# lawfuyang/ToyRenderer

Hardware: AMD Instinct MI355X
Metric: Gmeshlets/s culled (whole node), 100M meshlets (higher is better)
Workload: dtype f32

## Files before the change

toyrenderer_amd/csrc/host/nvrhi_lite.h:

```cpp
#pragma once

#include "HostProfile.h"

#include <atomic>
#include <cstdint>
#include <cstdio>
#include <cstdlib>
#include <memory>
#include <stdexcept>
#include <string>
#include <utility>
#include <vector>

#include "../../../include/trhip.h"

#define check(expr)                                                                          \
    do {                                                                                     \
        if (!(expr)) {                                                                       \
            std::fprintf(stderr, "check failed: %s (%s:%d)\n", #expr, __FILE__, __LINE__);   \
            std::abort();                                                                    \
        }                                                                                    \
    } while (0)

namespace nvrhi
// ... 316 lines not shown
    }
    void setPushConstants(const void* data, size_t bytes) { m_Push.assign((const uint8_t*)data, (const uint8_t*)data + bytes); }
    void dispatch(uint32_t gx, uint32_t gy = 1, uint32_t gz = 1)
    {
        std::vector<trhip_binding> b = flatten();
        HOST_PROFILE_SCOPE("trhip_cmd_dispatch (record)");
        throwIfFailed(trhip_cmd_dispatch(m_Native, m_State.pipeline.c_str(), b.data(), (uint32_t)b.size(),
                                         m_Push.empty() ? nullptr : m_Push.data(), (uint32_t)m_Push.size(), gx, gy, gz), "ICommandList::dispatch");
        m_Push.clear();
    }
    void dispatchIndirect(uint32_t offsetBytes)
    {
        check(m_State.indirectParams);
        std::vector<trhip_binding> b = flatten();
        HOST_PROFILE_SCOPE("trhip_cmd_dispatch_indirect (record)");
        throwIfFailed(trhip_cmd_dispatch_indirect(m_Native, m_State.pipeline.c_str(), b.data(), (uint32_t)b.size(),
                                                  m_Push.empty() ? nullptr : m_Push.data(), (uint32_t)m_Push.size(),
                                                  m_State.indirectParams->native(), offsetBytes), "ICommandList::dispatchIndirect");
        m_Push.clear();
    }
    void beginTimerQuery(ITimerQuery* q) { keep(q); throwIfFailed(trhip_cmd_begin_timer(m_Native, q->native()), "ICommandList::beginTimerQuery"); }
    void endTimerQuery(ITimerQuery* q) { q->m_Recorded = true; throwIfFailed(trhip_cmd_end_timer(m_Native, q->native()), "ICommandList::endTimerQuery"); }
    void beginPipelineStatisticsQuery(IPipelineStatisticsQuery* q) { keep(q); throwIfFailed(trhip_cmd_begin_pipeline_stats(m_Native, q->native()), "ICommandList::beginPipelineStatisticsQuery"); }
    void endPipelineStatisticsQuery(IPipelineStatisticsQuery* q) { q->m_Recorded = true; throwIfFailed(trhip_cmd_end_pipeline_stats(m_Native, q->native()), "ICommandList::endPipelineStatisticsQuery"); }
    void beginMarker(const char* name) { throwIfFailed(trhip_cmd_begin_marker(m_Native, name), "ICommandList::beginMarker"); }
    void endMarker() { throwIfFailed(trhip_cmd_end_marker(m_Native), "ICommandList::endMarker"); }

private:
    void keep(IResource* r) { if (r) m_Keep.emplace_back(r); }
    std::vector<trhip_binding> flatten() const
    {
        std::vector<trhip_binding> out;
        out.reserve(m_State.bindings.bindings.size());
        for (const BindingSetItem& i : m_State.bindings.bindings) {
            trhip_binding b{};
            b.type = i.type; b.slot = i.slot; b.baseMip = i.baseMip;
            if (i.buffer) b.resource = i.buffer->native();
            else if (i.texture) b.resource = i.texture->native();
            else if (i.table) b.resource = i.table->native();
            out.push_back(b);
        }
        return out;
    }

    trhip_cmdlist m_Native;
    ComputeState m_State;
    std::vector<uint8_t> m_Push;
    std::vector<ResourceHandle> m_Keep;
};
using CommandListHandle = RefCountPtr<ICommandList>;

namespace utils
{
struct ScopedMarker
{
    ScopedMarker(ICommandList* cl, const char* name) : m_Cl(cl) { m_Cl->beginMarker(name); }
    ~ScopedMarker() { m_Cl->endMarker(); }
    ICommandList* m_Cl;
};
}

class IDevice : public IResource
{
public:
    explicit IDevice(trhip_device d) : m_Native(d) {}
    ~IDevice() override { destroyQueues(); trhip_device_destroy(m_Native); }
    trhip_device native() const { return m_Native; }
    trhip_device queueDevice(CommandQueue queue)
    {
        if (queue != CommandQueue::Compute) return m_Native;
        if (!m_ComputeNative) {
            throwIfFailed(trhip_stream_create(m_DeviceIndex, &m_ComputeStream), "IDevice: compute-queue stream");
            throwIfFailed(trhip_device_create_on_stream(m_DeviceIndex, m_ComputeStream, &m_ComputeNative), "IDevice: compute-queue device");
        }
        return m_ComputeNative;
    }

    HeapHandle createHeap(const HeapDesc& d)
    {
        trhip_heap h = nullptr;
        throwIfFailed(trhip_heap_create(m_Native, d.capacity, &h), "IDevice::createHeap");
        return HeapHandle(new IHeap(h, d));
    }
    BufferHandle createBuffer(const BufferDesc& d)
    {
        trhip_buffer_desc n{};
        n.byteSize = d.byteSize; n.structStride = d.structStride; n.canHaveUAVs = d.canHaveUAVs; n.isDrawIndirectArgs = d.isDrawIndirectArgs;
        n.isVirtual = d.isVirtual; n.isVolatileConstant = d.isVolatile && d.isConstantBuffer; n.debugName = d.debugName.c_str();
        trhip_buffer b = nullptr;
        throwIfFailed(trhip_buffer_create(m_Native, &n, &b), "IDevice::createBuffer");
        return BufferHandle(new IBuffer(b, d));
    }
    TextureHandle createTexture(const TextureDesc& d)
    {
        trhip_texture_desc n{};
        n.width = d.width; n.height = d.height; n.mipLevels = d.mipLevels; n.isUAV = (d.isUAV ? 1u : 0u) | (d.isRenderTarget ? TRHIP_TEXTURE_RENDER_TARGET : 0u); n.isVirtual = d.isVirtual; n.debugName = d.debugName.c_str();
        n.format = d.format == Format::R16_FLOAT ? TRHIP_FORMAT_R16_FLOAT : d.format == Format::RG32_UINT ? TRHIP_FORMAT_RG32_UINT
                 : d.format == Format::RG16_FLOAT ? TRHIP_FORMAT_RG16_FLOAT : d.format == Format::RGBA32_UINT ? TRHIP_FORMAT_RGBA32_UINT
                 : d.format == Format::R11G11B10_FLOAT ? TRHIP_FORMAT_R11G11B10_FLOAT : d.format == Format::R8_UNORM ? TRHIP_FORMAT_R8_UNORM
                 : d.format == Format::R8_UINT ? TRHIP_FORMAT_R8_UINT : d.format == Format::RGBA8_UNORM ? TRHIP_FORMAT_RGBA8_UNORM
                 : d.format == Format::SRGBA8_UNORM ? TRHIP_FORMAT_SRGBA8_UNORM : d.format == Format::R10G10B10A2_UNORM ? TRHIP_FORMAT_R10G10B10A2_UNORM
                 : d.format == Format::RGBA16_FLOAT ? TRHIP_FORMAT_RGBA16_FLOAT : TRHIP_FORMAT_R32_FLOAT;
        trhip_texture t = nullptr;
        if (d.dimension == kTexture2DArray) throwIfFailed(trhip_texture_create_array(m_Native, &n, d.arraySize, &t), "IDevice::createTexture (array)");
        else throwIfFailed(trhip_texture_create(m_Native, &n, &t), "IDevice::createTexture");
        return TextureHandle(new ITexture(t, d));
    }
    SamplerHandle createSampler(const SamplerDesc& d) { return SamplerHandle(new ISampler(d)); }
    DescriptorTableHandle createDescriptorTable(uint32_t capacity)
    {
        trhip_texture_table t = nullptr;
        throwIfFailed(trhip_texture_table_create(m_Native, capacity, &t), "IDevice::createDescriptorTable");
        return DescriptorTableHandle(new IDescriptorTable(t));
    }
    void writeDescriptorTable(IDescriptorTable* table, uint32_t index, ITexture* t) { throwIfFailed(trhip_texture_table_set(table->native(), index, t->native()), "IDevice::writeDescriptorTable"); }
    MemoryRequirements getBufferMemoryRequirements(IBuffer* b)
    {
        MemoryRequirements r;
        throwIfFailed(trhip_buffer_memory_requirements(b->native(), &r.size, &r.alignment), "IDevice::getBufferMemoryRequirements");
        return r;
    }
    MemoryRequirements getTextureMemoryRequirements(ITexture* t)
    {
        MemoryRequirements r;
        throwIfFailed(trhip_texture_memory_requirements(t->native(), &r.size, &r.alignment), "IDevice::getTextureMemoryRequirements");
        return r;
    }
    bool bindBufferMemory(IBuffer* b, IHeap* h, uint64_t off) { throwIfFailed(trhip_buffer_bind_memory(b->native(), h->native(), off), "IDevice::bindBufferMemory"); return true; }
    bool bindTextureMemory(ITexture* t, IHeap* h, uint64_t off) { throwIfFailed(trhip_texture_bind_memory(t->native(), h->native(), off), "IDevice::bindTextureMemory"); return true; }
    CommandListHandle createCommandList(CommandQueue queue = CommandQueue::Graphics)
    {
        trhip_cmdlist cl = nullptr;
        throwIfFailed(trhip_cmd_create(queueDevice(queue), &cl), "IDevice::createCommandList");
        return CommandListHandle(new ICommandList(cl, queue));
    }
    uint64_t executeCommandLists(ICommandList* const* lists, size_t n, CommandQueue queue = CommandQueue::Graphics)
    {
        std::vector<trhip_cmdlist> v;
        for (size_t i = 0; i < n; ++i) { check(lists[i]->m_Queue == queue); v.push_back(lists[i]->native()); }
        throwIfFailed(trhip_queue_execute(queueDevice(queue), v.data(), (uint32_t)v.size()), "IDevice::executeCommandLists");
        return ++m_LastInstance[(size_t)queue];
    }
    uint64_t executeCommandList(ICommandList* cl) { return executeCommandLists(&cl, 1, cl->m_Queue); }
    void queueWaitForCommandList(CommandQueue waitQueue, CommandQueue executionQueue, uint64_t instance)
    {
        if (waitQueue == executionQueue) return;
        check(instance == m_LastInstance[(size_t)executionQueue]);
        trhip_device producer = queueDevice(executionQueue);
        void*& ev = m_QueueEvents[(size_t)executionQueue][instance % kQueueEvents];
        if (!ev) throwIfFailed(trhip_event_create(m_DeviceIndex, &ev), "IDevice::queueWaitForCommandList: event");
        throwIfFailed(trhip_device_join_side_stream(producer), "IDevice::queueWaitForCommandList: join");
        throwIfFailed(trhip_event_record(ev, trhip_device_stream(producer)), "IDevice::queueWaitForCommandList: record");
        throwIfFailed(trhip_stream_wait_event(trhip_device_stream(queueDevice(waitQueue)), ev), "IDevice::queueWaitForCommandList: wait");
    }
    uint64_t lastInstance(CommandQueue queue) const { return m_LastInstance[(size_t)queue]; }
    bool hasComputeQueue() const { return m_ComputeNative != nullptr; }
    void setDeviceIndex(int index) { m_DeviceIndex = index; }
    void waitForIdle()
    {
        throwIfFailed(trhip_device_wait_idle(m_Native), "IDevice::waitForIdle");
        if (m_ComputeNative) throwIfFailed(trhip_device_wait_idle(m_ComputeNative), "IDevice::waitForIdle (compute queue)");
    }
    void destroyQueues()
    {
        for (auto& q : m_QueueEvents) for (void*& e : q) { if (e) trhip_event_destroy(e); e = nullptr; }
        if (m_ComputeNative) { trhip_device_destroy(m_ComputeNative); m_ComputeNative = nullptr; }
        if (m_ComputeStream) { trhip_stream_destroy(m_ComputeStream); m_ComputeStream = nullptr; }
    }
    void runGarbageCollection() {}
    TimerQueryHandle createTimerQuery()
    {
        trhip_timer t = nullptr;
        throwIfFailed(trhip_timer_create(m_Native, &t), "IDevice::createTimerQuery");
        return TimerQueryHandle(new ITimerQuery(t));
    }
    float getTimerQueryTime(ITimerQuery* q)
    {
        if (!q || !q->m_Recorded) return 0.0f;
        float ms = 0.0f;
        if (trhip_timer_get_ms(q->native(), &ms) != TRHIP_OK) return 0.0f;
        return ms * 1e-3f;
    }
    void resetTimerQuery(ITimerQuery* q) { if (q) q->m_Recorded = false; }
    PipelineStatisticsQueryHandle createPipelineStatisticsQuery()
    {
        trhip_pipeline_stats q = nullptr;
        throwIfFailed(trhip_pipeline_stats_create(m_Native, &q), "IDevice::createPipelineStatisticsQuery");
        return PipelineStatisticsQueryHandle(new IPipelineStatisticsQuery(q));
    }
    PipelineStatistics getPipelineStatistics(IPipelineStatisticsQuery* q)
    {
        PipelineStatistics s;
        if (!q || !q->m_Recorded) return s;
        if (trhip_pipeline_stats_get(q->native(), reinterpret_cast<trhip_pipeline_statistics*>(&s)) != TRHIP_OK) return PipelineStatistics{};
        return s;
    }

private:
    static constexpr size_t kQueueEvents = 16;
    trhip_device m_Native;
    trhip_device m_ComputeNative = nullptr;
    void* m_ComputeStream = nullptr;
    int m_DeviceIndex = 0;
    uint64_t m_LastInstance[(size_t)CommandQueue::Count] = {};
    void* m_QueueEvents[(size_t)CommandQueue::Count][kQueueEvents] = {};
};
using DeviceHandle = RefCountPtr<IDevice>;

}
```

toyrenderer_amd/csrc/instance_cache.hip.h:

```cpp
#pragma once

#include <hip/hip_runtime.h>

#include "ShaderInterop.h"

struct InstanceCullCache
{
    const float4* sphere;
    const float4* world;
    const float* maxScale;
    const uint32_t* numLODs;
    const uint2* lodInfo;
    const float* error;
    const float4* localSphere;
    uint64_t stride;

    __host__ __device__ const uint2& lod(uint32_t id, uint32_t l) const { return lodInfo[(uint64_t)l * stride + id]; }
    __host__ __device__ const float& err(uint32_t id, uint32_t l) const { return error[(uint64_t)l * stride + id]; }
};

constexpr uint64_t kInstanceCacheBytesPerInstance = 64 + 16 + 4 + 4 + 3 * 4 * interop::kMaxNumMeshLODs + 16;

inline InstanceCullCache instanceCacheLayout(void* base, uint64_t n)
{
    char* p = (char*)base;
    InstanceCullCache c;
    c.world = (const float4*)p;             p += 64 * n;
    c.sphere = (const float4*)p;            p += 16 * n;
    c.maxScale = (const float*)p;           p += 4 * n;
    c.numLODs = (const uint32_t*)p;         p += 4 * n;
    c.lodInfo = (const uint2*)p;            p += 8ull * interop::kMaxNumMeshLODs * n;
    c.error = (const float*)p;              p += 4ull * interop::kMaxNumMeshLODs * n;
    c.localSphere = (const float4*)p;
    c.stride = n;
    return c;
}

__device__ __forceinline__ void instanceCacheWriteTransformPart(const InstanceCullCache& c, uint32_t i, float4 w0, float4 w1, float4 w2, float4 w3, float4 sph,
                                                                float4* worldOut = nullptr)
{
    const cm::M43 W = { { w0.x, w0.y, w0.z }, { w1.x, w1.y, w1.z }, { w2.x, w2.y, w2.z }, { w3.x, w3.y, w3.z } };
    const float ms = cm::maxScale(W.r0, W.r1, W.r2);
    const cm::F3 wc = cm::mulPoint({ sph.x, sph.y, sph.z }, W);
    const_cast<float4*>(c.sphere)[i] = make_float4(wc.x, wc.y, wc.z, sph.w * ms);
    float4* wr = worldOut ? worldOut : const_cast<float4*>(c.world) + 4ull * i;
    wr[0] = make_float4(w0.x, w0.y, w0.z, w1.x);
    wr[1] = make_float4(w1.y, w1.z, w2.x, w2.y);
    wr[2] = make_float4(w2.z, w3.x, w3.y, w3.z);
    wr[3] = make_float4(ms, 0.f, 0.f, 0.f);
    const_cast<float*>(c.maxScale)[i] = ms;
}
```

toyrenderer_amd/csrc/k_basepass_as.hip:

```cpp
#include <algorithm>
#include <cstdlib>
#include <string>
#include <type_traits>

#if defined(TR_STAMPS) || defined(TR_COUNT_SLOW) || defined(TR_COUNT_PATHS)
__device__ unsigned long long g_stampSums[8];
#define g_pathCount (g_stampSums + 4)
#endif
#include <atomic>
#include <memory>
#include <mutex>
#include <unordered_map>

#include "cull_math.hip.h"
#include "instance_cache.hip.h"
#include "meshlet_exact.hip.h"
#include "trhip_internal.h"

using namespace interop;

namespace
{

constexpr uint32_t kBlock = 256;
// ... 1101 lines not shown

void emitListBuild(const trhip::DispatchCtx& ctx, const MeshletCullArgs& a, const char* prefix, bool side, const void* argsBase)
{
    auto emit = [&](const std::string& name, std::function<int(hipStream_t)> fn) {
        if (side) ctx.emitSide(name.c_str(), std::move(fn), { { a.listGroups ? (const void*)a.listGroups : argsBase, false }, { a.visMask, false }, { a.visibleList, true }, { a.drawArgs, true } });
        else ctx.emit(name.c_str(), std::move(fn));
    };
    if (!side && a.recordCapacity <= kCompactMaxTiles * kCompactTile) {
        const uint32_t tiles = (a.recordCapacity + kCompactTile - 1) / kCompactTile;
        const size_t words = (size_t)kCompactMaxTiles * kStatusStride * 2 + 4;
        uint32_t* mem = (uint32_t*)ctx.scratch(words * 4);
        if (mem && ctx.cl->recordClearWords(mem, words, 0, true) == TRHIP_OK) {
            unsigned long long* status = (unsigned long long*)mem;
            uint32_t* ticket = mem + kCompactMaxTiles * kStatusStride * 2;
            uint32_t grid = ctx.computeUnits();
            if (grid > tiles) grid = tiles;
            if (grid == 0) grid = 1;
            emit(std::string(prefix) + "compact", [a, status, ticket, grid](hipStream_t s) {
                TRHIP_LAUNCH(visCompactKernel, dim3(grid), dim3(kCompactThreads), 0, s, a, status, ticket);
                return trhip::launchStatus("visCompactKernel"); });
            return;
        }
    }
    const uint32_t needBlocks = (a.maxBatches + kWaves - 1) / kWaves;
    uint32_t gridSmall = ctx.computeUnits() * 8u;
    if (gridSmall > needBlocks) gridSmall = needBlocks;
    if (gridSmall == 0) gridSmall = 1;
    const std::string p = prefix;
    const uint32_t supers = (a.maxBatches >> kSuperShift) + 1u;
    emit(p + "count", [a, supers](hipStream_t s) {
        TRHIP_LAUNCH(visCountKernel, dim3(supers), dim3(kCountThreads), 0, s, a);
        return trhip::launchStatus("visCountKernel"); });
    emit(p + "scan", [a](hipStream_t s) {
        TRHIP_LAUNCH(visSuperScanKernel, dim3(1), dim3(1024), 0, s, a);
        return trhip::launchStatus("visSuperScanKernel"); });
    emit(p + "expand", [a, gridSmall](hipStream_t s) {
        TRHIP_LAUNCH(visExpandKernel, dim3(gridSmall), dim3(kBlock), 0, s, a);
        return trhip::launchStatus("visExpandKernel"); });
}

template <bool F, bool O, bool C>
void launchCull(const MeshletCullArgs& a, uint32_t grid, bool table, hipStream_t s)
{
    if (O && table) TRHIP_LAUNCH((meshletCullKernel<F, O, C, true>), dim3(grid), dim3(kCullBlock), 0, s, a);
    else TRHIP_LAUNCH((meshletCullKernel<F, O, C, false>), dim3(grid), dim3(kCullBlock), 0, s, a);
}

constexpr uint64_t kStreamBytesPerMeshlet = 20;
__host__ __device__ inline MeshletCullStream meshletStreamLayout(void* mem, uint64_t numMeshlets)
{
    const uint64_t coneAt = (numMeshlets * 16u + 255u) & ~255ull;
    return { reinterpret_cast<const float4*>(mem), reinterpret_cast<const uint32_t*>(reinterpret_cast<char*>(mem) + coneAt) };
}
inline uint64_t meshletStreamBytes(uint64_t numMeshlets) { return ((numMeshlets * 16u + 255u) & ~255ull) + numMeshlets * 4u; }

__global__ __launch_bounds__(256) void meshletStreamKernel(const MeshletData* __restrict__ meshlets, uint64_t n, MeshletCullStream out)
{
    const uint64_t stride = (uint64_t)gridDim.x * 256u;
    for (uint64_t i = (uint64_t)blockIdx.x * 256u + threadIdx.x; i < n; i += stride) {
        const float4* p = reinterpret_cast<const float4*>(meshlets + i);
        const float4 sphere = p[0];
        const uint32_t cone = __float_as_uint(p[1].x);
        const_cast<float4*>(out.sphere)[i] = sphere;
        const_cast<uint32_t*>(out.cone)[i] = cone;
    }
}

int meshletStreamLaunchBuild(trhip_buffer_t* meshlets, hipStream_t s)
{
    const trhip::Stamp from = { meshlets->version };
    if (meshlets->cullStream.current(from)) return TRHIP_OK;
    const uint64_t n = meshlets->byteSize / sizeof(MeshletData);
    const uint64_t blocks = (n + 255u) / 256u;
    TRHIP_LAUNCH(meshletStreamKernel, dim3((uint32_t)(blocks < 65536u ? (blocks ? blocks : 1u) : 65536u)), dim3(256), 0, s,
                       (const MeshletData*)meshlets->ptr, n, meshletStreamLayout(meshlets->cullStream.ptr, n));
    meshlets->cullStream.markBuilt(from);
    return trhip::launchStatus("meshletStreamKernel");
}

int recordASMain(trhip::DispatchCtx& ctx)
{
    const BasePassConstants* k = (const BasePassConstants*)ctx.constants(0, sizeof(BasePassConstants));
    TRHIP_REQUIRE(k, "%s: constant buffer b0 (BasePassConstants, 256 bytes) missing", ctx.shaderName);
    trhip_buffer_t* instances = ctx.buffer(TRHIP_BIND_STRUCTURED_SRV, 0);
    trhip_buffer_t* meshData = ctx.buffer(TRHIP_BIND_STRUCTURED_SRV, 2);
    trhip_buffer_t* meshlets = ctx.buffer(TRHIP_BIND_STRUCTURED_SRV, 4);
    trhip_buffer_t* records = ctx.buffer(TRHIP_BIND_STRUCTURED_SRV, 7);
    trhip_texture_t* hzb = ctx.texture(TRHIP_BIND_TEXTURE_SRV, 8);
    trhip_buffer_t* visMask = ctx.buffer(TRHIP_BIND_STRUCTURED_UAV, 0);
    trhip_buffer_t* visList = ctx.buffer(TRHIP_BIND_STRUCTURED_UAV, 1);
    trhip_buffer_t* drawArgs = ctx.buffer(TRHIP_BIND_STRUCTURED_UAV, 2);
    TRHIP_REQUIRE(instances && meshData && meshlets && records, "%s: needs SRVs t0, t2, t4, t7 (BasePassRenderers.cpp:463-479)", ctx.shaderName);
    TRHIP_REQUIRE(visMask && visList && drawArgs, "%s: needs UAVs u0 (visMask), u1 (visibleList), u2 (drawArgs)", ctx.shaderName);
    TRHIP_REQUIRE(ctx.indirect, "%s: launched by dispatchMeshIndirect (BasePassRenderers.cpp:497-502): use dispatch_indirect", ctx.shaderName);
    TRHIP_REQUIRE(instances->byteSize % sizeof(BasePassInstanceConstants) == 0, "%s: instance buffer size is not a multiple of 144", ctx.shaderName);
    TRHIP_REQUIRE(meshlets->byteSize % sizeof(MeshletData) == 0, "%s: meshlet buffer size is not a multiple of 32", ctx.shaderName);
    TRHIP_REQUIRE(drawArgs->byteSize >= 12, "%s: drawArgs buffer smaller than 12 bytes", ctx.shaderName);

    MeshletCullArgs a;
    memset(&a, 0, sizeof a);
    a.k = *k;
    const bool occlusion = (k->m_CullingFlags & kCullingFlagOcclusionCullingEnable) != 0;
    const bool useTable = occlusion && ctx.variant == 0 && records->byteSize / sizeof(MeshletAmplificationData) >= trhip::tableMinGroups();
    int rc = TRHIP_OK;
    {
        memset(&a.hzb, 0, sizeof a.hzb);
        if (occlusion) {
            TRHIP_REQUIRE(hzb, "%s: occlusion culling enabled but no HZB texture bound at t8", ctx.shaderName);
            TRHIP_REQUIRE(hzb->format == TRHIP_FORMAT_R16_FLOAT, "%s: HZB is not R16_FLOAT", ctx.shaderName);
            TRHIP_REQUIRE(hzb->width == k->m_HZBDimensions.x && hzb->height == k->m_HZBDimensions.y,
                          "%s: m_HZBDimensions %ux%u does not match the HZB texture %ux%u", ctx.shaderName,
                          k->m_HZBDimensions.x, k->m_HZBDimensions.y, hzb->width, hzb->height);
            a.hzb.base = (const _Float16*)hzb->ptr;
            a.hzb.width = hzb->width; a.hzb.height = hzb->height; a.hzb.mips = hzb->mips;
            for (uint32_t m = 0; m < hzb->mips; ++m) a.hzb.mipOffset[m] = (uint32_t)(hzb->mipOffset[m] / 2);
            if (useTable) {
                rc = trhip::hzbQuadEnsure(hzb);
                if (rc != TRHIP_OK) return rc;
                a.quad.base = (const _Float16*)hzb->quad.ptr;
                a.quad.total = hzb->quadTotal;
                for (uint32_t m = 0; m < hzb->mips; ++m) a.quad.offset[m] = hzb->quadOffset[m];
            }
        }
    }
    if (rc != TRHIP_OK) return rc;
    a.meshlets = (const MeshletData*)meshlets->ptr;
    TRHIP_REQUIRE(meshlets->byteSize >= sizeof(MeshletData), "%s: empty meshlet buffer", ctx.shaderName);
    rc = meshlets->cullStream.allocate(meshlets->dev, meshletStreamBytes(meshlets->byteSize / sizeof(MeshletData)));
    if (rc != TRHIP_OK) return rc;
    a.stream = meshletStreamLayout(meshlets->cullStream.ptr, meshlets->byteSize / sizeof(MeshletData));
    a.records = (const MeshletAmplificationData*)records->ptr;
    a.dispatchArgs = (const uint32_t*)((const char*)ctx.argsBuffer->ptr + ctx.argsOffset);
    a.argsWords = (ctx.argsBuffer->byteSize - ctx.argsOffset) >= 16 ? 4u : 3u;
    const uint64_t cap = records->byteSize / sizeof(MeshletAmplificationData);
    a.recordCapacity = cap > 0xFFFFFFFFull ? 0xFFFFFFFFu : (uint32_t)cap;
    TRHIP_REQUIRE(a.recordCapacity <= (1u << 27), "%s: more than 2^27 records cannot be encoded as (g<<5)|lane", ctx.shaderName);
    TRHIP_REQUIRE(visMask->byteSize / 4 >= a.recordCapacity, "%s: visMask holds %llu groups, records buffer %u", ctx.shaderName,
                  (unsigned long long)(visMask->byteSize / 4), a.recordCapacity);
    a.numMeshlets = meshlets->byteSize / sizeof(MeshletData);
    TRHIP_REQUIRE(a.numMeshlets <= (1ull << 32), "%s: more than 2^32 meshlets (m_MeshletDataBufferIdx is 32 bits wide)", ctx.shaderName);
    a.visMask = (uint32_t*)visMask->ptr;
    a.visibleList = (uint32_t*)visList->ptr;
    const uint64_t lcap = visList->byteSize / 4;
    a.listCapacity = lcap > 0xFFFFFFFFull ? 0xFFFFFFFFu : (uint32_t)lcap;
    a.drawArgs = (uint32_t*)drawArgs->ptr;
    if (records->order.ptr && records->order.bytes >= 256 + (uint64_t)a.recordCapacity * 16) {
        a.permHeader = (const uint32_t*)records->order.ptr;
        a.perm = (const uint4*)(a.permHeader + 64);
    }
    rc = trhip::instanceCacheEnsure(instances);
    if (rc != TRHIP_OK) return rc;
    a.numInstances = (uint32_t)(instances->byteSize / sizeof(BasePassInstanceConstants));
    a.cache = instanceCacheLayout(instances->cullCache.ptr, a.numInstances);
    a.maxBatches = (a.recordCapacity + kBatch - 1) / kBatch;
    a.batchSum = (uint32_t*)(a.recordCapacity >= (1u << 19) ? ctx.scratchSide((size_t)a.maxBatches * 4)
                                                            : ctx.scratch((size_t)a.maxBatches * 4));
    TRHIP_REQUIRE(a.batchSum, "%s: scratch allocation failed", ctx.shaderName);
    {
        const size_t supers = (a.maxBatches >> kSuperShift) + 1u;
        a.superSum = (uint32_t*)(a.recordCapacity >= (1u << 19) ? ctx.scratchSide(supers * 4) : ctx.scratch(supers * 4));
        TRHIP_REQUIRE(a.superSum, "%s: scratch allocation failed", ctx.shaderName);
    }

    const uint32_t blocksPerCU = TR_CULL_WAVES_PER_EU;
    uint32_t grid = ctx.computeUnits() * blocksPerCU;
    const uint32_t needBlocks = (a.recordCapacity + kCullBatch * kCullWaves - 1) / (kCullBatch * kCullWaves);
    if (grid > needBlocks) grid = needBlocks;
    if (grid == 0) grid = 1;
    rc = visMask->listCount.allocate(visMask->dev, 256);
    if (rc != TRHIP_OK) return rc;
    a.listGroups = (uint32_t*)visMask->listCount.ptr;
    ctx.cl->use(a.listGroups, ctx.cl->ops.size(), true);
    if (useTable) a.bands = cm::projBands(k->m_P00, k->m_P11, hzb->width, hzb->height);
    static const bool noShortPass = getenv("TRHIP_NO_SHORT_PASS") != nullptr;
    a.shortPassRounds = noShortPass ? 0u : kShortPassRounds;
    const uint32_t flags = k->m_CullingFlags & 7u;
    trhip_texture_t* quadOwner = useTable ? hzb : nullptr;
    const bool table = useTable;
    if (quadOwner) ctx.cl->use(quadOwner->quad.ptr, ctx.cl->ops.size(), false);
    ctx.emit("cull", [a, grid, flags, quadOwner, table, instances, meshData, meshlets](hipStream_t s) {
        if ((const void*)a.meshlets != meshlets->ptr)
            return trhip::fail(TRHIP_ERR_STATE, "basepass_AS_Main: the meshlet buffer was bound to other memory after this command list was recorded: record it again");
        {
            int crc = trhip::instanceCacheLaunchBuild(instances, meshData, s);
            if (crc != TRHIP_OK) return crc;
            crc = meshletStreamLaunchBuild(meshlets, s);
            if (crc != TRHIP_OK) return crc;
        }
        if (quadOwner) {
            int brc = trhip::hzbQuadLaunchBuild(quadOwner, s);
            if (brc != TRHIP_OK) return brc;
        }
        switch (flags) {
        case 0: launchCull<false, false, false>(a, grid, table, s); break;
        case 1: launchCull<true, false, false>(a, grid, table, s); break;
        case 2: launchCull<false, true, false>(a, grid, table, s); break;
        case 3: launchCull<true, true, false>(a, grid, table, s); break;
        case 4: launchCull<false, false, true>(a, grid, table, s); break;
        case 5: launchCull<true, false, true>(a, grid, table, s); break;
        case 6: launchCull<false, true, true>(a, grid, table, s); break;
        default: launchCull<true, true, true>(a, grid, table, s); break;
        }
        return trhip::launchStatus("meshletCullKernel"); });
    emitListBuild(ctx, a, "", a.recordCapacity >= (1u << 19), ctx.argsBuffer->ptr);
    if (ctx.cl->openStats)
        return trhip::statsEmitAS(ctx, a, meshlets, records, instances, meshData, a.recordCapacity >= (1u << 19));
    return TRHIP_OK;
}

int recordPackShard(trhip::DispatchCtx& ctx)
{
    const uint32_t* push = (const uint32_t*)ctx.constants(0, 8);
    trhip_buffer_t* slot = ctx.buffer(TRHIP_BIND_STRUCTURED_UAV, 0);
    trhip_buffer_t* state = ctx.buffer(TRHIP_BIND_STRUCTURED_UAV, 1);
    TRHIP_REQUIRE(push && slot && state, "%s: needs push constants {slotGroups, slotRuns}, UAV u0 (shard slot) and UAV u1 (state words, zeroed once)", ctx.shaderName);
    ShardPackArgs a;
    memset(&a, 0, sizeof a);
    a.slotGroups = push[0];
    a.slotRuns = push[1];
    const uint64_t slotWords = (uint64_t)kSlotHeaderWords + 4ull * a.slotRuns + a.slotGroups;
    TRHIP_REQUIRE(slot->byteSize >= slotWords * 4, "%s: shard slot buffer smaller than 16 + 4 * %u + %u words", ctx.shaderName, a.slotRuns, a.slotGroups);
    const uint64_t maxTiles = (uint64_t)a.slotGroups / kPackTile + kMaxPassSlots + 1u;
    TRHIP_REQUIRE(maxTiles < (1u << 30) && state->byteSize >= maxTiles * 16u, "%s: state buffer u1 smaller than %llu bytes", ctx.shaderName, (unsigned long long)(maxTiles * 16u));
    TRHIP_REQUIRE(((uintptr_t)slot->ptr & 15u) == 0 && ((uintptr_t)state->ptr & 7u) == 0, "%s: u0 / u1 not 16 / 8-byte aligned", ctx.shaderName);
    a.slot = (uint32_t*)slot->ptr;
    a.maxTiles = (uint32_t)maxTiles;
    unsigned long long* halves = (unsigned long long*)state->ptr;
    for (uint32_t s = 0; s < kMaxPassSlots; ++s) {
        trhip_buffer_t* rec = ctx.buffer(TRHIP_BIND_STRUCTURED_SRV, 4 * s);
        trhip_buffer_t* mask = ctx.buffer(TRHIP_BIND_STRUCTURED_SRV, 4 * s + 1);
        trhip_buffer_t* args = ctx.buffer(TRHIP_BIND_STRUCTURED_SRV, 4 * s + 2);
        trhip_buffer_t* draw = ctx.buffer(TRHIP_BIND_STRUCTURED_SRV, 4 * s + 3);
        if (!rec && !mask && !args && !draw) continue;
        TRHIP_REQUIRE(rec && mask && args && draw, "%s: pass slot %u needs t%u..t%u (records, visMask, dispatch args, draw args)", ctx.shaderName, s, 4 * s, 4 * s + 3);
        TRHIP_REQUIRE(args->byteSize >= 12 && draw->byteSize >= 12, "%s: argument buffers smaller than 12 bytes", ctx.shaderName);
        const uint64_t cap = std::min<uint64_t>(rec->byteSize / sizeof(MeshletAmplificationData), mask->byteSize / 4);
        a.records[s] = (const uint32_t*)rec->ptr;
        a.masks[s] = (const uint32_t*)mask->ptr;
        a.dispatchArgs[s] = (const uint32_t*)args->ptr;
        a.drawArgs[s] = (const uint32_t*)draw->ptr;
        a.argsWords[s] = args->byteSize >= 16 ? 4u : 3u;
        a.recordCapacity[s] = cap > 0xFFFFFFFFull ? 0xFFFFFFFFu : (uint32_t)cap;
    }
    a.tileBlocks = (uint32_t)std::min<uint64_t>(maxTiles, (uint64_t)ctx.computeUnits() * 3u);
    const uint32_t maskBlocks = (uint32_t)std::min<uint64_t>(std::max<uint64_t>(((uint64_t)a.slotGroups + 4u * kPackThreads - 1u) / (4u * kPackThreads), 1u), ctx.computeUnits());
    const uint32_t grid = a.tileBlocks + maskBlocks;
    static std::mutex mu;
    static std::unordered_map<void*, std::shared_ptr<std::atomic<uint32_t>>> launches;
    std::shared_ptr<std::atomic<uint32_t>> count;
    {
        std::lock_guard<std::mutex> lock(mu);
        std::shared_ptr<std::atomic<uint32_t>>& c = launches[(void*)halves];
        if (!c) c = std::make_shared<std::atomic<uint32_t>>(0u);
        count = c;
    }
    ctx.emit("main", [a, grid, halves, count](hipStream_t s) {
        ShardPackArgs l = a;
        const uint32_t half = count->fetch_add(1u) & 1u;
        l.status = halves + (size_t)half * a.maxTiles;
        l.statusNext = halves + (size_t)(half ^ 1u) * a.maxTiles;
        TRHIP_LAUNCH(shardPackKernel, dim3(grid), dim3(kPackThreads), 0, s, l);
        return trhip::launchStatus("shardPackKernel"); });
    return TRHIP_OK;
}

int recordUnpackShards(trhip::DispatchCtx& ctx)
{
    const uint32_t* push = (const uint32_t*)ctx.constants(0, 12);
    trhip_buffer_t* recv = ctx.buffer(TRHIP_BIND_STRUCTURED_SRV, 0);
    TRHIP_REQUIRE(push && recv, "%s: needs push constants {world, slotGroups, slotRuns[, globalGroupCapacity]} and SRV t0 (gathered slots)", ctx.shaderName);
    ShardUnpackArgs a;
    memset(&a, 0, sizeof a);
    a.world = push[0];
    a.slotGroups = push[1];
    a.slotRuns = push[2];
    if (const uint32_t* push4 = (const uint32_t*)ctx.constants(0, 16)) a.globalCap = push4[3];
    TRHIP_REQUIRE(a.world >= 1 && a.world <= kMaxRanks, "%s: world size %u outside [1, %u]", ctx.shaderName, a.world, kMaxRanks);
    const uint64_t words = (uint64_t)a.world * (kSlotHeaderWords + 4ull * a.slotRuns + a.slotGroups);
    TRHIP_REQUIRE(words < (1ull << 32), "%s: %u slots of %u groups / %u runs exceed 2^32 words", ctx.shaderName, a.world, a.slotGroups, a.slotRuns);
    TRHIP_REQUIRE(recv->byteSize >= words * 4, "%s: gathered buffer smaller than world x slot", ctx.shaderName);
    TRHIP_REQUIRE(((uintptr_t)recv->ptr & 15u) == 0, "%s: t0 not 16-byte aligned", ctx.shaderName);
    a.recv = (const uint32_t*)recv->ptr;
    MeshletCullArgs lists[kMaxPassSlots];
    uint64_t copyWords = 0;
    for (uint32_t s = 0; s < kMaxPassSlots; ++s) {
        trhip_buffer_t* rec = ctx.buffer(TRHIP_BIND_STRUCTURED_UAV, 4 * s);
        trhip_buffer_t* mask = ctx.buffer(TRHIP_BIND_STRUCTURED_UAV, 4 * s + 1);
        trhip_buffer_t* list = ctx.buffer(TRHIP_BIND_STRUCTURED_UAV, 4 * s + 2);
        trhip_buffer_t* args = ctx.buffer(TRHIP_BIND_STRUCTURED_UAV, 4 * s + 3);
        if (!rec && !mask && !list && !args) continue;
        TRHIP_REQUIRE(rec && mask && list && args, "%s: pass slot %u needs u%u..u%u (records, masks, visible list, args)", ctx.shaderName, s, 4 * s, 4 * s + 3);
        TRHIP_REQUIRE(args->byteSize >= 32, "%s: args buffer of pass slot %u smaller than 32 bytes", ctx.shaderName, s);
        const uint64_t cap = std::min<uint64_t>(rec->byteSize / sizeof(MeshletAmplificationData), mask->byteSize / 4);
        TRHIP_REQUIRE(cap <= (1u << 27), "%s: more than 2^27 records cannot be encoded as (g<<5)|lane", ctx.shaderName);
        a.records[s] = (uint32_t*)rec->ptr;
        a.masks[s] = (uint32_t*)mask->ptr;
        a.args[s] = (uint32_t*)args->ptr;
        a.capacity[s] = (uint32_t)cap;
        copyWords += std::min<uint64_t>(cap, (uint64_t)a.world * a.slotGroups);
        MeshletCullArgs& l = lists[s];
        memset(&l, 0, sizeof l);
        l.dispatchArgs = a.args[s];
        l.argsWords = 4;
        l.recordCapacity = a.capacity[s];
        l.visMask = a.masks[s];
        l.visibleList = (uint32_t*)list->ptr;
        const uint64_t lcap = list->byteSize / 4;
        l.listCapacity = lcap > 0xFFFFFFFFull ? 0xFFFFFFFFu : (uint32_t)lcap;
        l.drawArgs = a.args[s] + 4;
        l.maxBatches = (l.recordCapacity + kBatch - 1) / kBatch;
        l.batchSum = (uint32_t*)ctx.scratch((size_t)l.maxBatches * 4);
        const size_t supers = (l.maxBatches >> kSuperShift) + 1u;
        l.superSum = (uint32_t*)ctx.scratch(supers * 4);
        TRHIP_REQUIRE(l.batchSum && l.superSum, "%s: scratch allocation failed", ctx.shaderName);

    }
    uint32_t grid = ctx.computeUnits() * 4u;
    const uint64_t need = (copyWords + 255u) / 256u;
    if (grid > need) grid = (uint32_t)need;
    if (grid == 0) grid = 1;
    ctx.emit("unpack", [a, grid](hipStream_t s) {
        TRHIP_LAUNCH(shardUnpackKernel, dim3(grid), dim3(256), 0, s, a);
        return trhip::launchStatus("shardUnpackKernel"); });
    for (uint32_t s = 0; s < kMaxPassSlots; ++s)
        if (a.records[s]) {
            const char prefix[] = { 's', 'l', 'o', 't', (char)('0' + s), '_', 0 };
            emitListBuild(ctx, lists[s], prefix, false, nullptr);
        }
    return TRHIP_OK;
}

trhip::ShaderRegistrar rp("visibility_CS_PackShard", recordPackShard, 0);
trhip::ShaderRegistrar ru("visibility_CS_UnpackShards", recordUnpackShards, 0);
// ... 18 lines not shown
```

toyrenderer_amd/csrc/k_gpuculling.hip:

```cpp
#include "cull_math.hip.h"
#include "hzb_quad.hip.h"
#include "instance_cache.hip.h"
#include "trhip_internal.h"

using namespace interop;

namespace
{

constexpr uint32_t kBlock = 256;
constexpr uint32_t kWordSubmit = 1u << 30;
constexpr uint32_t kWordLate = 1u << 31;
constexpr uint32_t kGroupMask = (1u << 27) - 1u;

struct InstanceCullArgs
{
    GPUCullingPassConstants k;
    const BasePassInstanceConstants* instances;
    const uint32_t* ids;
    const MeshData* meshData;
    cm::Hzb hzb;
    MeshletAmplificationData* records;
    uint32_t* dispatchArgs;
    uint32_t* lateCount;
    uint32_t* lateIds;
    const uint32_t* indirectArgs;
    InstanceCullCache cache;
    uint32_t numInstances;
    const uint32_t* shardLate;
    uint32_t directThreads;
    uint32_t maxGroups;
    uint32_t argsWords;
    uint32_t* word;
    uint32_t* localOff;
    uint32_t* blockGroups;
    uint64_t* blockLateSubmit;
    uint32_t* bases;
    uint32_t numBlocks;
    uint32_t* tileHist;
    uint32_t* tileTotal;
    uint16_t* tileOf;
    uint2* lodSel;
    uint32_t* permHeader;
    uint4* perm;
    uint32_t permCapacity;
    uint32_t* lateArgsOut;
    unsigned long long* fusedStatus;
    uint32_t* fusedTicket;
};

struct QuadShare { bool stale = false; };
struct EarlyCullNote { InstanceCullArgs a; size_t scanOp; bool fused; trhip_texture_t* quadOwner = nullptr; std::shared_ptr<QuadShare> share; };

__global__ __launch_bounds__(256) void instanceCacheKernel(const BasePassInstanceConstants* instances, uint32_t n,
                                                           const MeshData* meshData, uint32_t numMeshes, InstanceCullCache c)
{
    const uint32_t i = blockIdx.x * 256u + threadIdx.x;
    if (i >= n) return;
    const BasePassInstanceConstants& inst = instances[i];
    const float4 w0 = *reinterpret_cast<const float4*>(inst.m_WorldMatrix.m[0]);
    const float4 w1 = *reinterpret_cast<const float4*>(inst.m_WorldMatrix.m[1]);
    const float4 w2 = *reinterpret_cast<const float4*>(inst.m_WorldMatrix.m[2]);
    const float4 w3 = *reinterpret_cast<const float4*>(inst.m_WorldMatrix.m[3]);
    const uint32_t meshIdx = inst.m_MeshDataIdx;
    float4 sph = make_float4(0.f, 0.f, 0.f, 0.f);
    uint32_t numLODs = 0;
    uint32_t nm[kMaxNumMeshLODs], mb[kMaxNumMeshLODs];
    float err[kMaxNumMeshLODs];
#pragma unroll
    for (uint32_t l = 0; l < kMaxNumMeshLODs; ++l) { nm[l] = 0; mb[l] = 0; err[l] = 0.f; }
    if (meshIdx < numMeshes) {
        const MeshData& mesh = meshData[meshIdx];
        sph = *reinterpret_cast<const float4*>(&mesh.m_BoundingSphere);
        numLODs = mesh.m_NumLODs;
#pragma unroll
        for (uint32_t l = 0; l < kMaxNumMeshLODs; ++l) {
            nm[l] = mesh.m_MeshLODDatas[l].m_NumMeshlets; mb[l] = mesh.m_MeshLODDatas[l].m_MeshletDataBufferIdx; err[l] = mesh.m_MeshLODDatas[l].m_Error;
        }
    }
    instanceCacheWriteTransformPart(c, i, w0, w1, w2, w3, sph);
    const_cast<float4*>(c.localSphere)[i] = sph;
    const_cast<uint32_t*>(c.numLODs)[i] = numLODs;
#pragma unroll
    for (uint32_t l = 0; l < kMaxNumMeshLODs; ++l) {
        const_cast<uint2&>(c.lod(i, l)) = make_uint2(nm[l], mb[l]);
        const_cast<float&>(c.err(i, l)) = err[l];
    }
}

#ifndef TR_TILES_PER_AXIS
#define TR_TILES_PER_AXIS 16
#endif
constexpr uint32_t kTilesPerAxis = TR_TILES_PER_AXIS;
constexpr uint32_t kNumTiles = kTilesPerAxis * kTilesPerAxis;
constexpr uint32_t kPermHeaderWords = 64;
#ifndef TR_MIN_BINNED
#define TR_MIN_BINNED 4096
#endif
constexpr uint32_t kMinBinnedEntries = TR_MIN_BINNED;

__device__ __forceinline__ uint32_t screenTile(cm::F3 cv, float P00, float P11)
{
    const float iz = __builtin_amdgcn_rcpf(cm::max_(cv.z, 1e-6f));
    const float u = cm::fma_(cv.x * iz * P00, 0.5f, 0.5f), v = cm::fma_(cv.y * iz * P11, -0.5f, 0.5f);
    const int tx = min(max((int)(u * (float)kTilesPerAxis), 0), (int)kTilesPerAxis - 1);
    const int ty = min(max((int)(v * (float)kTilesPerAxis), 0), (int)kTilesPerAxis - 1);
    return (uint32_t)ty * kTilesPerAxis + (uint32_t)tx;
}

template <int LATE>
__device__ __forceinline__ uint32_t threadCount(const InstanceCullArgs& a)
{
    if (LATE) {
        uint32_t count = *a.lateCount;
        uint64_t launched = (uint64_t)a.indirectArgs[0] * kNumThreadsPerWave;
        if (a.shardLate) {
            const uint64_t all = (((uint64_t)a.shardLate[1] + 63u) / 64u) * kNumThreadsPerWave;
            launched = all > a.shardLate[0] ? all - a.shardLate[0] : 0u;
        }
        uint32_t n = launched < count ? (uint32_t)launched : count;
        return n < a.k.m_NbInstances ? n : a.k.m_NbInstances;
    }
    return a.directThreads < a.k.m_NbInstances ? a.directThreads : a.k.m_NbInstances;
}

__device__ __forceinline__ uint32_t waveInclusiveScan(uint32_t v, uint32_t lane)
{
#pragma unroll
    for (int d = 1; d < 64; d <<= 1) {
        uint32_t n = __shfl_up(v, d);
        if (lane >= (uint32_t)d) v += n;
    }
    return v;
}

template <int LATE>
__device__ __forceinline__ uint32_t classify(const InstanceCullArgs& a, uint32_t id, uint32_t* tileOut, uint2* lodOut)
{
    const GPUCullingPassConstants& k = a.k;
    const bool doFrustum = (k.m_CullingFlags & kCullingFlagFrustumCullingEnable) != 0;
    const bool doOcclusion = (k.m_CullingFlags & kCullingFlagOcclusionCullingEnable) != 0;

    const uint32_t cid = id < a.numInstances ? id : 0u;
    const float4 ws = a.cache.sphere[cid];
    const float ms = a.cache.maxScale[cid];
    const cm::F3 wc = { ws.x, ws.y, ws.z };
    const float r = ws.w;
    cm::F3 cv = cm::toView(wc, cm::loadM43(k.m_WorldToView));

    if (!LATE && doFrustum &&
        !cm::frustumVisible(cv, r, k.m_Frustum.x, k.m_Frustum.y, k.m_Frustum.z, k.m_Frustum.w))
        return 0;

    if (doOcclusion) {
        if (!LATE) cv = cm::toView(wc, cm::loadM43(k.m_PrevWorldToView));
        if (!cm::occlusionVisible(cv, r, k.m_NearPlane, k.m_P00, k.m_P11, a.hzb))
            return LATE ? 0 : kWordLate;
    }

    const uint32_t numLODs = a.cache.numLODs[cid];
    uint32_t lod = 0;
    if (k.m_ForcedMeshLOD != kInvalidMeshLOD) {
        const uint32_t last = numLODs - 1u;
        lod = k.m_ForcedMeshLOD < last ? k.m_ForcedMeshLOD : last;
    } else {
        const float distance = cm::max_(cm::sqrt_(cm::dot3(cv, cv)) - r, 0.0f);
        const float threshold = distance * k.m_MeshLODTarget / ms;
        const uint32_t n = numLODs < kMaxNumMeshLODs ? numLODs : kMaxNumMeshLODs;
        for (uint32_t i = 1; i < n; ++i)
            if (a.cache.err(cid, i) < threshold) lod = i;
    }
    lod = lod < kMaxNumMeshLODs ? lod : kMaxNumMeshLODs - 1u;
    const uint2 li = a.cache.lod(cid, lod);
    *lodOut = li;
    const uint32_t numMeshlets = li.x;
    const uint32_t groups = (numMeshlets + kNumThreadsPerWave - 1u) / kNumThreadsPerWave;
    *tileOut = screenTile(cv, k.m_P00, k.m_P11);
    return kWordSubmit | (lod << 27) | (groups & kGroupMask);
}

#ifndef TR_BIG_THREADS
#define TR_BIG_THREADS 512
#endif
#ifndef TR_BIG_PER
#define TR_BIG_PER 1
#endif
constexpr uint32_t kBigThreads = TR_BIG_THREADS;
constexpr uint32_t kBigPerThread = TR_BIG_PER;
constexpr uint32_t kScanThreads = 1024;
constexpr uint32_t kBigChunk = kBigThreads * kBigPerThread;
constexpr uint32_t kBigWaves = kBigThreads / 64;
constexpr uint32_t kScanTilesPerGroup = kNumTiles < 16 ? kNumTiles : 16;
constexpr uint32_t kScanTileGroups = kNumTiles / kScanTilesPerGroup;
constexpr uint32_t kScanStripes = kScanThreads / kScanTilesPerGroup;

template <int LATE>
__device__ __forceinline__ uint32_t activeBigBlocks(const InstanceCullArgs& a, uint32_t n)
{
    const uint32_t need = (n + kBigChunk - 1) / kBigChunk;
    return need < a.numBlocks ? need : a.numBlocks;
}

// ... 269 lines not shown
constexpr uint32_t kFusedLateMaxTiles = 4096;
constexpr uint32_t kFusedStatusStride = 16;
constexpr unsigned long long kFusedFlag = 1ull << 63, kFusedPoison = 1ull << 60;

template <int LATE>
__global__ __launch_bounds__(kBlock) void instanceFusedKernel(InstanceCullArgs a, trhip::QuadArgs q)
{
    if (!LATE && blockIdx.x >= a.numBlocks) {
        __shared__ float s_t[9][trhip::kQuadStripCols + 1];
        trhip::hzbQuadStrip(q, blockIdx.x - a.numBlocks, s_t);
        return;
    }
    __shared__ uint32_t s_waveG[kBlock / 64], s_waveL[kBlock / 64], s_waveS[kBlock / 64];
    __shared__ unsigned long long s_preG[kBlock / 64], s_preLS[kBlock / 64];
    __shared__ uint32_t s_tile;
    const uint32_t n = threadCount<LATE>(a);
    const uint32_t numTiles = (n + kBlock - 1) / kBlock < a.numBlocks ? (n + kBlock - 1) / kBlock : a.numBlocks;
    const uint32_t tid = threadIdx.x, lane = tid & 63u, wave = tid >> 6;
    const uint32_t baseX = __hip_atomic_load(&a.dispatchArgs[0], __ATOMIC_RELAXED, __HIP_MEMORY_SCOPE_AGENT);
    const uint32_t baseLate = LATE ? 0u : __hip_atomic_load(a.lateCount, __ATOMIC_RELAXED, __HIP_MEMORY_SCOPE_AGENT);
    if (blockIdx.x >= (numTiles ? numTiles : 1u)) return;
    {
        if (tid == 0) s_tile = atomicAdd(a.fusedTicket, 1u);
        __syncthreads();
        const uint32_t tile = s_tile;
        const uint32_t t = tile * kBlock + tid;
        uint32_t word = 0, tileUnused = 0;
        uint2 lodUnused;
        if (t < n) word = classify<LATE>(a, a.ids[t], &tileUnused, &lodUnused);
        const uint32_t g = (word & kWordSubmit) ? (word & kGroupMask) : 0u;
        const uint32_t late = word >> 31;
        const uint32_t submit = (word >> 30) & 1u;
        const uint32_t incG = waveInclusiveScan(g, lane);
        const uint32_t incL = waveInclusiveScan(late, lane);
        const uint32_t cntS = (uint32_t)__popcll(__ballot(submit != 0));
        if (lane == 63) { s_waveG[wave] = incG; s_waveL[wave] = incL; s_waveS[wave] = cntS; }
        __syncthreads();
        uint32_t baseG = 0, baseL = 0, totG = 0, totL = 0, totS = 0;
#pragma unroll
        for (uint32_t w = 0; w < kBlock / 64; ++w) {
            if (w < wave) { baseG += s_waveG[w]; baseL += s_waveL[w]; }
            totG += s_waveG[w]; totL += s_waveL[w]; totS += s_waveS[w];
        }
        const uint32_t localOff = late ? (baseL + incL - late) : (baseG + incG - g);
        unsigned long long* line = a.fusedStatus + (uint64_t)tile * kFusedStatusStride;
        if (tid == 0 && numTiles != 0) {
            __hip_atomic_store(&line[0], kFusedFlag | (unsigned long long)totG, __ATOMIC_RELAXED, __HIP_MEMORY_SCOPE_AGENT);
            __hip_atomic_store(&line[1], kFusedFlag | ((unsigned long long)totS << 32) | (unsigned long long)totL, __ATOMIC_RELAXED, __HIP_MEMORY_SCOPE_AGENT);
        }
        unsigned long long sumG = 0, sumLS = 0;
        for (uint32_t j = tid; j < tile; j += kBlock) {
            const unsigned long long* pl = a.fusedStatus + (uint64_t)j * kFusedStatusStride;
            unsigned long long v0 = 0, v1 = 0;
            uint32_t spins = 0;
            for (;;) {
                v0 = __hip_atomic_load(&pl[0], __ATOMIC_RELAXED, __HIP_MEMORY_SCOPE_AGENT);
                v1 = __hip_atomic_load(&pl[1], __ATOMIC_RELAXED, __HIP_MEMORY_SCOPE_AGENT);
                if ((v0 & v1 & kFusedFlag) != 0ull) { v0 &= ~kFusedFlag; v1 &= ~kFusedFlag; break; }
                if (++spins > (1u << 22)) { v0 = kFusedPoison; v1 = 0; break; }
                __builtin_amdgcn_s_sleep(1);
            }
            sumG += v0; sumLS += v1;
        }
#pragma unroll
        for (int d = 32; d >= 1; d >>= 1) { sumG += __shfl_xor(sumG, d); sumLS += __shfl_xor(sumLS, d); }
        if (lane == 0) { s_preG[wave] = sumG; s_preLS[wave] = sumLS; }
        __syncthreads();
        unsigned long long preG = 0, preLS = 0;
#pragma unroll
        for (uint32_t w = 0; w < kBlock / 64; ++w) { preG += s_preG[w]; preLS += s_preLS[w]; }
        const uint32_t prefixG = (uint32_t)preG, prefixL = (uint32_t)preLS;
        if (t < n) {
            if (word & kWordLate) {
                a.lateIds[baseLate + prefixL + localOff] = a.ids[t];
            } else if (word & kWordSubmit) {
                const uint32_t groups = word & kGroupMask;
                const uint32_t lod = (word >> 27) & 7u;
                const uint32_t off = baseX + prefixG + localOff;
                if (off + groups >= a.maxGroups) {
                    if (groups != 0 && off < a.maxGroups && a.argsWords > 3) a.dispatchArgs[3] = off;
                } else {
                    const uint32_t id = a.ids[t];
                    for (uint32_t i = 0; i < groups; ++i) {
                        MeshletAmplificationData rec = { id, lod, i * kNumThreadsPerWave };
                        a.records[off + i] = rec;
                    }
                }
            }
        }
        if (tid == 0 && (tile == numTiles - 1u || numTiles == 0)) {
            const unsigned long long allG = preG + totG;
            const uint32_t allL = prefixL + totL, allS = (uint32_t)(preLS >> 32) + totS;
            const uint32_t X = (allG >> 40) ? 0xFFFFFFFFu : baseX + (uint32_t)allG;
            a.bases[0] = baseX;
            a.bases[1] = baseLate;
            a.dispatchArgs[0] = X;
            if (allS != 0) { a.dispatchArgs[1] = 1; a.dispatchArgs[2] = 1; }
            if (a.argsWords > 3 && (X < a.maxGroups || baseX >= a.maxGroups)) a.dispatchArgs[3] = X;
            if (!LATE) {
                const uint32_t lateTotal = baseLate + allL;
                *a.lateCount = lateTotal;
                if (a.lateArgsOut) { a.lateArgsOut[0] = (lateTotal + 63u) / 64u; a.lateArgsOut[1] = 1; a.lateArgsOut[2] = 1; }
            }
            a.permHeader[0] = 0u;
            a.permHeader[1] = X;
        }
    }
}

__global__ void buildLateCullIndirectArgsKernel(const uint32_t* count, uint32_t* args)
{
    args[0] = (count[0] + 63u) / 64u;
    args[1] = 1;
    args[2] = 1;
}

__global__ void shardLateInfoKernel(const uint32_t* counts, uint32_t world, uint32_t rank, uint32_t* info)
{
    uint32_t below = 0, all = 0;
    for (uint32_t p = 0; p < world; ++p) {
        const uint32_t c = counts[p];
        if (p < rank) below += c;
        all += c;
    }
    info[0] = below;
    info[1] = all;
}

int fillHzb(const trhip::DispatchCtx& ctx, trhip_texture_t* tex, const Vector2U& dims, bool occlusion, cm::Hzb* out)
{
    memset(out, 0, sizeof *out);
    if (!occlusion) return TRHIP_OK;
    TRHIP_REQUIRE(tex, "%s: occlusion culling enabled but no HZB texture bound", ctx.shaderName);
    TRHIP_REQUIRE(tex->format == TRHIP_FORMAT_R16_FLOAT, "%s: HZB '%s' is not R16_FLOAT", ctx.shaderName, tex->name.c_str());
    TRHIP_REQUIRE(tex->width == dims.x && tex->height == dims.y,
                  "%s: m_HZBDimensions %ux%u does not match HZB texture %ux%u", ctx.shaderName, dims.x, dims.y, tex->width, tex->height);
    out->base = (const _Float16*)tex->ptr;
    out->width = tex->width; out->height = tex->height; out->mips = tex->mips;
    for (uint32_t k = 0; k < tex->mips; ++k) out->mipOffset[k] = (uint32_t)(tex->mipOffset[k] / 2);
    return TRHIP_OK;
}

std::function<int(hipStream_t)> fusedEarlyLaunch(const InstanceCullArgs& a, trhip_texture_t* quadOwner)
{
    return [a, quadOwner](hipStream_t s) {
        trhip::QuadArgs q;
        memset(&q, 0, sizeof q);
        uint32_t strips = 0;
        if (quadOwner && !quadOwner->quad.current({ quadOwner->version })) {
            q = trhip::quadArgs(quadOwner);
            strips = q.firstStrip[q.mips];
            quadOwner->quad.markBuilt({ quadOwner->version });
        }
        TRHIP_LAUNCH(instanceFusedKernel<0>, dim3(a.numBlocks + strips), dim3(kBlock), 0, s, a, q);
        return trhip::launchStatus("instanceFusedKernel"); };
}

inline uint32_t quadScanStrips(uint32_t all)
{
    static const uint32_t pct = [] { const char* e = getenv("TRHIP_QUAD_SCAN_PERCENT"); const int v = e ? atoi(e) : 50; return (uint32_t)(v < 0 ? 0 : v > 100 ? 100 : v); }();
    return (uint32_t)((uint64_t)all * pct / 100u);
}

std::function<int(hipStream_t)> scanEarlyLaunch(const InstanceCullArgs& a, trhip_texture_t* quadOwner, std::shared_ptr<QuadShare> share)
{
    return [a, quadOwner, share](hipStream_t s) {
        trhip::QuadArgs q;
        memset(&q, 0, sizeof q);
        uint32_t extra = 0, stripEnd = 0;
        if (share) share->stale = false;
        if (quadOwner && !quadOwner->quad.current({ quadOwner->version })) {
            q = trhip::quadArgs(quadOwner);
            stripEnd = share ? quadScanStrips(q.firstStrip[q.mips]) : q.firstStrip[q.mips];
            extra = (stripEnd + kScanStripsPerGroup - 1u) / kScanStripsPerGroup;
            quadOwner->quad.markBuilt({ quadOwner->version });
            if (share) share->stale = true;
        }
        TRHIP_LAUNCH(instanceScanKernel<0>, dim3(1 + kScanTileGroups + extra), dim3(kScanThreads), 0, s, a, q, stripEnd);
        return trhip::launchStatus("instanceScanKernel"); };
}

template <int LATE>
int recordGPUCulling(trhip::DispatchCtx& ctx)
{
    const GPUCullingPassConstants* k = (const GPUCullingPassConstants*)ctx.constants(0, sizeof(GPUCullingPassConstants));
    TRHIP_REQUIRE(k, "%s: constant buffer b0 (GPUCullingPassConstants, 180 bytes) missing", ctx.shaderName);
    trhip_buffer_t* instances = ctx.buffer(TRHIP_BIND_STRUCTURED_SRV, 0);
    trhip_buffer_t* ids = ctx.buffer(TRHIP_BIND_STRUCTURED_SRV, 1);
    trhip_buffer_t* meshData = ctx.buffer(TRHIP_BIND_STRUCTURED_SRV, 2);
    trhip_texture_t* hzb = ctx.texture(TRHIP_BIND_TEXTURE_SRV, 3);
    trhip_buffer_t* records = ctx.buffer(TRHIP_BIND_STRUCTURED_UAV, 0);
    trhip_buffer_t* args = ctx.buffer(TRHIP_BIND_STRUCTURED_UAV, 1);
    trhip_buffer_t* lateCount = ctx.buffer(TRHIP_BIND_STRUCTURED_UAV, 2);
    trhip_buffer_t* lateIds = ctx.buffer(TRHIP_BIND_STRUCTURED_UAV, 3);
    trhip_buffer_t* shardLate = LATE ? ctx.buffer(TRHIP_BIND_STRUCTURED_SRV, 4) : nullptr;
    TRHIP_REQUIRE(!shardLate || shardLate->byteSize >= 8, "%s: shard late info (t4) smaller than 8 bytes", ctx.shaderName);
    TRHIP_REQUIRE(instances && ids && meshData && records && args && lateCount && lateIds,
                  "%s: needs SRVs t0..t2 and UAVs u0..u3 (BasePassRenderers.cpp:351-362)", ctx.shaderName);
    const bool occlusion = (k->m_CullingFlags & kCullingFlagOcclusionCullingEnable) != 0;
    TRHIP_REQUIRE(instances->byteSize % sizeof(BasePassInstanceConstants) == 0, "%s: instance buffer size is not a multiple of 144", ctx.shaderName);
    TRHIP_REQUIRE(meshData->byteSize % sizeof(MeshData) == 0, "%s: mesh data buffer size is not a multiple of 156", ctx.shaderName);
    TRHIP_REQUIRE(records->byteSize >= sizeof(MeshletAmplificationData), "%s: amplification buffer too small", ctx.shaderName);
    TRHIP_REQUIRE(args->byteSize >= 12, "%s: dispatch-arguments buffer smaller than 12 bytes", ctx.shaderName);
    if (LATE) {
        TRHIP_REQUIRE(ctx.indirect, "%s: LATE_CULL=1 is dispatched indirectly (BasePassRenderers.cpp:399)", ctx.shaderName);
        TRHIP_REQUIRE(occlusion, "%s: LATE_CULL=1 without occlusion culling", ctx.shaderName);
        TRHIP_REQUIRE((uint64_t)k->m_NbInstances * 4 <= lateIds->byteSize, "%s: late id buffer smaller than m_NbInstances", ctx.shaderName);
    } else {
        TRHIP_REQUIRE(!ctx.indirect, "%s: LATE_CULL=0 is dispatched directly", ctx.shaderName);
        TRHIP_REQUIRE((uint64_t)k->m_NbInstances * 4 <= ids->byteSize, "%s: m_NbInstances %u exceeds the id buffer", ctx.shaderName, k->m_NbInstances);
        if (occlusion)
            TRHIP_REQUIRE((uint64_t)k->m_NbInstances * 4 <= lateIds->byteSize, "%s: late id buffer smaller than m_NbInstances", ctx.shaderName);
    }
    TRHIP_REQUIRE(lateCount->byteSize >= 4, "%s: late counter buffer too small", ctx.shaderName);

    InstanceCullArgs a;
    memset(&a, 0, sizeof a);
    a.k = *k;
    int rc = fillHzb(ctx, hzb, k->m_HZBDimensions, occlusion, &a.hzb);
    if (rc != TRHIP_OK) return rc;
    a.instances = (const BasePassInstanceConstants*)instances->ptr;
    a.ids = LATE ? (const uint32_t*)lateIds->ptr : (const uint32_t*)ids->ptr;
    a.meshData = (const MeshData*)meshData->ptr;
    a.records = (MeshletAmplificationData*)records->ptr;
    a.dispatchArgs = (uint32_t*)args->ptr;
    a.lateCount = (uint32_t*)lateCount->ptr;
    a.lateIds = (uint32_t*)lateIds->ptr;
    a.indirectArgs = LATE ? (const uint32_t*)((const char*)ctx.argsBuffer->ptr + ctx.argsOffset) : nullptr;
    a.shardLate = shardLate ? (const uint32_t*)shardLate->ptr : nullptr;
    const uint64_t direct = (uint64_t)ctx.gx * kNumThreadsPerWave;
    a.directThreads = direct > 0xFFFFFFFFull ? 0xFFFFFFFFu : (uint32_t)direct;
    const uint64_t cap = records->byteSize / sizeof(MeshletAmplificationData);
    a.maxGroups = cap > 0xFFFFFFFFull ? 0xFFFFFFFFu : (uint32_t)cap;
    a.argsWords = args->byteSize >= 16 ? 4u : 3u;

    const uint32_t nMax = k->m_NbInstances;
    if (nMax == 0) return TRHIP_OK;

    rc = trhip::instanceCacheEnsure(instances);
    if (rc != TRHIP_OK) return rc;
    a.cache = instanceCacheLayout(instances->cullCache.ptr, instances->byteSize / sizeof(BasePassInstanceConstants));
    a.numInstances = (uint32_t)(instances->byteSize / sizeof(BasePassInstanceConstants));
    ctx.emit("instance_cache", [instances, meshData](hipStream_t s) { return trhip::instanceCacheLaunchBuild(instances, meshData, s); });
    static const bool noFused = getenv("TRHIP_NO_FUSED_INSTANCE") != nullptr;
    const bool fusedPath = (nMax <= kFusedMaxEntries || (LATE && (nMax + kBlock - 1) / kBlock <= kFusedLateMaxTiles)) && !noFused;
    a.numBlocks = fusedPath ? (nMax + kBlock - 1) / kBlock : (nMax + kBigChunk - 1) / kBigChunk;
    a.word = (uint32_t*)ctx.scratch((size_t)nMax * 4);
    a.localOff = (uint32_t*)ctx.scratch((size_t)nMax * 4);
    a.blockGroups = (uint32_t*)ctx.scratch((size_t)a.numBlocks * 4);
    a.blockLateSubmit = (uint64_t*)ctx.scratch((size_t)a.numBlocks * 8);
    a.bases = (uint32_t*)ctx.scratch(16);
    a.tileHist = (uint32_t*)ctx.scratch(fusedPath ? 16 : (size_t)a.numBlocks * kNumTiles * 4);
    a.tileTotal = (uint32_t*)ctx.scratch(kNumTiles * 4);
    a.tileOf = (uint16_t*)ctx.scratch((size_t)nMax * 2);
    a.lodSel = (uint2*)ctx.scratch((size_t)nMax * 8);
    TRHIP_REQUIRE(a.word && a.localOff && a.blockGroups && a.blockLateSubmit && a.bases && a.tileHist && a.tileTotal && a.tileOf && a.lodSel, "%s: scratch allocation failed", ctx.shaderName);
    rc = records->order.allocate(records->dev, (uint64_t)kPermHeaderWords * 4 + (uint64_t)a.maxGroups * 16);
    if (rc != TRHIP_OK) return rc;
    a.permHeader = (uint32_t*)records->order.ptr;
    a.perm = (uint4*)(a.permHeader + kPermHeaderWords);
    a.permCapacity = a.maxGroups;
    const bool wantTable = !LATE && occlusion && a.maxGroups >= trhip::tableMinGroups();
    if (wantTable) {
        rc = trhip::hzbQuadEnsure(hzb);
        if (rc != TRHIP_OK) return rc;
    }

    if (fusedPath) {
        const size_t words = (size_t)a.numBlocks * kFusedStatusStride * 2 + 4;
        uint32_t* mem = (uint32_t*)ctx.scratch(words * 4);
        TRHIP_REQUIRE(mem, "%s: scratch allocation failed", ctx.shaderName);
        rc = ctx.cl->recordClearWords(mem, words, 0, true);
        if (rc != TRHIP_OK) return rc;
        a.fusedStatus = (unsigned long long*)mem;
        a.fusedTicket = mem + (size_t)a.numBlocks * kFusedStatusStride * 2;
        trhip_texture_t* quadOwner = wantTable ? hzb : nullptr;
        if (quadOwner) ctx.cl->use(quadOwner->quad.ptr, ctx.cl->ops.size(), true);
        if (LATE) ctx.emit("fused", [a](hipStream_t s) {
            trhip::QuadArgs q;
            memset(&q, 0, sizeof q);
            TRHIP_LAUNCH(instanceFusedKernel<LATE>, dim3(a.numBlocks), dim3(kBlock), 0, s, a, q);
            return trhip::launchStatus("instanceFusedKernel"); });
        else ctx.emit("fused", fusedEarlyLaunch(a, quadOwner));
        if (!LATE && occlusion) ctx.cl->peephole = { ctx.cl->ops.size() - 1, "gpuculling_early", std::make_shared<EarlyCullNote>(EarlyCullNote{ a, ctx.cl->ops.size() - 1, true, quadOwner }) };
        return TRHIP_OK;
    }

    ctx.emit("classify", [a](hipStream_t s) {
        TRHIP_LAUNCH(instanceClassifyKernel<LATE>, dim3(a.numBlocks), dim3(kBigThreads), 0, s, a);
        return trhip::launchStatus("instanceClassifyKernel"); });
    trhip_texture_t* quadOwner = wantTable ? hzb : nullptr;
    std::shared_ptr<QuadShare> share = quadOwner ? std::make_shared<QuadShare>() : nullptr;
    if (quadOwner) ctx.cl->use(quadOwner->quad.ptr, ctx.cl->ops.size(), true);
    if (LATE) ctx.emit("scan", [a](hipStream_t s) {
        trhip::QuadArgs q;
        memset(&q, 0, sizeof q);
        TRHIP_LAUNCH(instanceScanKernel<LATE>, dim3(1 + kScanTileGroups), dim3(kScanThreads), 0, s, a, q, 0u);
        return trhip::launchStatus("instanceScanKernel"); });
    else ctx.emit("scan", scanEarlyLaunch(a, quadOwner, share));
    const size_t scanOp = ctx.cl->ops.size() - 1;
    if (quadOwner) ctx.cl->use(quadOwner->quad.ptr, ctx.cl->ops.size(), true);
    ctx.emit("emit", [a, quadOwner, share](hipStream_t s) {
        trhip::QuadArgs q;
        memset(&q, 0, sizeof q);
        uint32_t extra = 0, stripBegin = 0;
        if (!LATE && quadOwner && share && share->stale) {
            q = trhip::quadArgs(quadOwner);
            stripBegin = quadScanStrips(q.firstStrip[q.mips]);
            extra = (q.firstStrip[q.mips] - stripBegin + kEmitStripsPerGroup - 1u) / kEmitStripsPerGroup;
        }
        TRHIP_LAUNCH(instanceEmitKernel<LATE>, dim3(a.numBlocks + extra), dim3(kBigThreads), 0, s, a, q, stripBegin);
        return trhip::launchStatus("instanceEmitKernel"); });
    if (!LATE && occlusion) ctx.cl->peephole = { ctx.cl->ops.size() - 1, "gpuculling_early", std::make_shared<EarlyCullNote>(EarlyCullNote{ a, scanOp, false, quadOwner, share }) };
    return TRHIP_OK;
}

int recordBuildLateArgs(trhip::DispatchCtx& ctx)
{
    trhip_buffer_t* count = ctx.buffer(TRHIP_BIND_STRUCTURED_SRV, 0);
    trhip_buffer_t* args = ctx.buffer(TRHIP_BIND_STRUCTURED_UAV, 0);
    TRHIP_REQUIRE(count && args, "%s: needs SRV t0 (late count) and UAV u0 (indirect args)", ctx.shaderName);
    TRHIP_REQUIRE(count->byteSize >= 4 && args->byteSize >= 12, "%s: buffers too small", ctx.shaderName);
    TRHIP_REQUIRE(!ctx.indirect && ctx.gx == 1 && ctx.gy == 1 && ctx.gz == 1, "%s: dispatched as 1x1x1", ctx.shaderName);
    const uint32_t* c = (const uint32_t*)count->ptr;
    uint32_t* a = (uint32_t*)args->ptr;
    const trhip_cmdlist_t::Peephole ph = ctx.cl->peephole;
    if (ph.kind && !strcmp(ph.kind, "gpuculling_early") && ph.op != SIZE_MAX && ph.op == ctx.cl->ops.size() - 1) {
        const EarlyCullNote* note = (const EarlyCullNote*)ph.data.get();
        if (note->a.lateCount == c && note->scanOp < ctx.cl->ops.size() && ctx.cl->ops[note->scanOp].lane == 0) {
            InstanceCullArgs fused = note->a;
            fused.lateArgsOut = a;
            const size_t scanOp = note->scanOp;
            if (note->fused) ctx.cl->ops[scanOp].fn = fusedEarlyLaunch(fused, note->quadOwner);
            else ctx.cl->ops[scanOp].fn = scanEarlyLaunch(fused, note->quadOwner, note->share);
            for (size_t i = ctx.cl->useMarks.size(); i-- > 0 && ctx.cl->useMarks[i].op >= ctx.cl->ops.size();) ctx.cl->useMarks[i].op = scanOp;
            ctx.cl->peephole = trhip_cmdlist_t::Peephole();
            return TRHIP_OK;
        }
    }
    ctx.emit("main", [c, a](hipStream_t s) {
        TRHIP_LAUNCH(buildLateCullIndirectArgsKernel, dim3(1), dim3(1), 0, s, c, a);
        return trhip::launchStatus("buildLateCullIndirectArgsKernel"); });
    return TRHIP_OK;
}

trhip::ShaderRegistrar r0("gpuculling_CS_GPUCulling LATE_CULL=0", recordGPUCulling<0>, 0);
trhip::ShaderRegistrar r1("gpuculling_CS_GPUCulling LATE_CULL=1", recordGPUCulling<1>, 1);
trhip::ShaderRegistrar r2("gpuculling_CS_BuildLateCullIndirectArgs", recordBuildLateArgs, 0);

}

namespace trhip
{

int instanceCacheEnsure(trhip_buffer_t* instances)
{
    const uint64_t n = instances->byteSize / sizeof(BasePassInstanceConstants);
    TRHIP_REQUIRE(n >= 1 && n <= 0xFFFFFFFFull, "instance cull cache: instance buffer '%s' size out of range", instances->name.c_str());
    return instances->cullCache.allocate(instances->dev, n * kInstanceCacheBytesPerInstance);
}

int instanceCacheLaunchBuild(trhip_buffer_t* instances, trhip_buffer_t* meshData, hipStream_t s)
{
    const Stamp from = { instances->version, meshData->ptr, meshData->version };
    if (instances->cullCache.current(from)) return TRHIP_OK;
    const uint32_t n = (uint32_t)(instances->byteSize / sizeof(BasePassInstanceConstants));
    const uint64_t numMeshes = meshData->byteSize / sizeof(MeshData);
    TRHIP_LAUNCH(instanceCacheKernel, dim3((n + 255u) / 256u), dim3(256), 0, s, (const BasePassInstanceConstants*)instances->ptr, n,
                       (const MeshData*)meshData->ptr, (uint32_t)(numMeshes > 0xFFFFFFFFull ? 0xFFFFFFFFull : numMeshes),
                       instanceCacheLayout(instances->cullCache.ptr, n));
    instances->cullCache.markBuilt(from);
    return launchStatus("instanceCacheKernel");
}

}

extern "C" int trhip_launch_shard_late_info(void* hip_stream, const uint32_t* gathered_counts, uint32_t world, uint32_t rank, uint32_t* info)
{
    if (!gathered_counts || !info || world == 0 || rank >= world)
        return trhip::fail(TRHIP_ERR_INVALID, "launch_shard_late_info: bad arguments (world %u, rank %u)", world, rank);
    TRHIP_LAUNCH(shardLateInfoKernel, dim3(1), dim3(1), 0, (hipStream_t)hip_stream, gathered_counts, world, rank, info);
    return trhip::launchStatus("shardLateInfoKernel");
}
```

toyrenderer_amd/csrc/k_updateinstance.hip:

```cpp
#include <cstddef>

#include "cull_math.hip.h"
#include "instance_cache.hip.h"
#include "trhip_internal.h"

using namespace interop;

namespace
{

struct M44 { float m[4][4]; };

__device__ __forceinline__ M44 matmul(const M44& A, const M44& B)
{
    M44 C;
#pragma unroll
    for (int i = 0; i < 4; ++i)
#pragma unroll
        for (int j = 0; j < 4; ++j)
            C.m[i][j] = cm::fma_(A.m[i][3], B.m[3][j], cm::fma_(A.m[i][2], B.m[2][j], cm::fma_(A.m[i][1], B.m[1][j], A.m[i][0] * B.m[0][j])));
    return C;
}

__device__ __forceinline__ M44 makeWorldMatrix(const NodeLocalTransform& t)
{
    const float qx = t.m_Rotation[0], qy = t.m_Rotation[1], qz = t.m_Rotation[2], qw = t.m_Rotation[3];
    const float qxx = qx * qx, qyy = qy * qy, qzz = qz * qz;
    M44 R = {}, S = {}, T = {};
    R.m[0][0] = (1.f - 2.f * qyy) - 2.f * qzz;
    R.m[0][1] = (2.f * qx) * qy + (2.f * qz) * qw;
    R.m[0][2] = (2.f * qx) * qz - (2.f * qy) * qw;
    R.m[1][0] = (2.f * qx) * qy - (2.f * qz) * qw;
    R.m[1][1] = (1.f - 2.f * qxx) - 2.f * qzz;
    R.m[1][2] = (2.f * qy) * qz + (2.f * qx) * qw;
    R.m[2][0] = (2.f * qx) * qz + (2.f * qy) * qw;
    R.m[2][1] = (2.f * qy) * qz - (2.f * qx) * qw;
    R.m[2][2] = (1.f - 2.f * qxx) - 2.f * qyy;
    R.m[3][3] = 1.f;
    S.m[0][0] = t.m_Scale[0]; S.m[1][1] = t.m_Scale[1]; S.m[2][2] = t.m_Scale[2]; S.m[3][3] = 1.f;
    T.m[0][0] = 1.f; T.m[1][1] = 1.f; T.m[2][2] = 1.f; T.m[3][3] = 1.f;
    T.m[3][0] = t.m_Position[0]; T.m[3][1] = t.m_Position[1]; T.m[3][2] = t.m_Position[2];
    return matmul(matmul(R, S), T);
}

#ifndef TR_UPD_BLOCK
#define TR_UPD_BLOCK 256
#endif
constexpr uint32_t kUpdBlock = TR_UPD_BLOCK;
constexpr uint32_t kRecVec = sizeof(BasePassInstanceConstants) / 16;
static_assert(sizeof(BasePassInstanceConstants) % 16 == 0 && offsetof(BasePassInstanceConstants, m_PrevWorldMatrix) == 64, "record layout");

__global__ __launch_bounds__(kUpdBlock) void updateInstanceConstsKernel(const NodeLocalTransform* __restrict__ nodes, uint32_t numNodes,
                                                                        const uint32_t* __restrict__ primToNode,
                                                                        BasePassInstanceConstants* instances, uint32_t first, uint32_t n,
                                                                        bool refreshCache, InstanceCullCache cache)
{
    __shared__ float4 s_rec[kUpdBlock * kRecVec];
    __shared__ float4 s_world[kUpdBlock * 4];
    const uint32_t tid = threadIdx.x;
    const uint32_t b0 = blockIdx.x * kUpdBlock;
    const uint32_t cnt = n - b0 < kUpdBlock ? n - b0 : kUpdBlock;
    const uint32_t i0 = first + b0;
    const uint32_t i = i0 + tid;
    const bool mine = tid < cnt;
    const uint32_t nodeID = mine ? primToNode[i] : 0xFFFFFFFFu;
    float4* g = reinterpret_cast<float4*>(instances + i0);
    float4 v[kRecVec];
#pragma unroll
    for (uint32_t k = 0; k < kRecVec; ++k) {
        const uint32_t e = k * kUpdBlock + tid;
        v[k] = e < cnt * kRecVec ? g[e] : make_float4(0.f, 0.f, 0.f, 0.f);
    }
    const bool valid = mine && nodeID < numNodes;
    NodeLocalTransform lt = {};
    float4 sph = make_float4(0.f, 0.f, 0.f, 0.f);
    if (valid) lt = nodes[nodeID];
    if (valid && refreshCache) sph = cache.localSphere[i];
#pragma unroll
    for (uint32_t k = 0; k < kRecVec; ++k) s_rec[k * kUpdBlock + tid] = v[k];
    M44 world = {};
    if (valid) {
        world = makeWorldMatrix(lt);
        uint32_t parent = lt.m_ParentNodeIdx;
        uint32_t guard = 0;
        while (parent != 0xFFFFFFFFu && parent < numNodes && guard++ < 1024) {
            const NodeLocalTransform pt = nodes[parent];
            world = matmul(world, makeWorldMatrix(pt));
            parent = pt.m_ParentNodeIdx;
        }
    }
    __syncthreads();
    if (valid) {
        float4* rec = s_rec + tid * kRecVec;
        float4 rows[4];
#pragma unroll
        for (int r = 0; r < 4; ++r) {
            rows[r] = make_float4(world.m[r][0], world.m[r][1], world.m[r][2], world.m[r][3]);
            rec[4 + r] = rec[r];
            rec[r] = rows[r];
        }
        if (refreshCache) instanceCacheWriteTransformPart(cache, i, rows[0], rows[1], rows[2], rows[3], sph, s_world + 4u * tid);
    }
    __syncthreads();
#pragma unroll
    for (uint32_t k = 0; k < kRecVec; ++k) {
        const uint32_t e = k * kUpdBlock + tid;
        if (e < cnt * kRecVec) g[e] = s_rec[e];
    }
    if (refreshCache) {
        float4* cw = const_cast<float4*>(cache.world) + 4ull * i0;
        const bool all = __syncthreads_and(valid || !mine) != 0;
        if (all) {
#pragma unroll
            for (uint32_t k = 0; k < 4; ++k) {
                const uint32_t e = k * kUpdBlock + tid;
                if (e < cnt * 4u) cw[e] = s_world[e];
            }
        } else if (valid) {
#pragma unroll
            for (uint32_t k = 0; k < 4; ++k) cw[4u * tid + k] = s_world[4u * tid + k];
        }
    }
}

int recordUpdateInstanceConsts(trhip::DispatchCtx& ctx)
{
    const UpdateInstanceConstsShardConstants* ks = (const UpdateInstanceConstsShardConstants*)ctx.constants(0, sizeof(UpdateInstanceConstsShardConstants));
    UpdateInstanceConstsShardConstants kk = { 0u, 0u };
    if (ks) kk = *ks;
    else if (const UpdateInstanceConstsPassConstants* k1 = (const UpdateInstanceConstsPassConstants*)ctx.constants(0, sizeof(UpdateInstanceConstsPassConstants))) kk.m_NumInstances = k1->m_NumInstances;
    else TRHIP_REQUIRE(false, "%s: push constants (UpdateInstanceConstsPassConstants) missing", ctx.shaderName);
    const UpdateInstanceConstsShardConstants* k = &kk;
    const uint32_t first = kk.m_FirstInstance;
    trhip_buffer_t* nodes = ctx.buffer(TRHIP_BIND_STRUCTURED_SRV, 0);
    trhip_buffer_t* primToNode = ctx.buffer(TRHIP_BIND_STRUCTURED_SRV, 1);
    trhip_buffer_t* instances = ctx.buffer(TRHIP_BIND_STRUCTURED_UAV, 0);
    TRHIP_REQUIRE(nodes && primToNode && instances, "%s: needs SRVs t0 (nodes), t1 (prim->node) and UAV u0 (instances)", ctx.shaderName);
    TRHIP_REQUIRE(nodes->byteSize % sizeof(NodeLocalTransform) == 0, "%s: node buffer size is not a multiple of 48", ctx.shaderName);
    TRHIP_REQUIRE(((uint64_t)first + k->m_NumInstances) * 4 <= primToNode->byteSize, "%s: the instance range exceeds the prim->node buffer", ctx.shaderName);
    TRHIP_REQUIRE(((uint64_t)first + k->m_NumInstances) * sizeof(BasePassInstanceConstants) <= instances->byteSize, "%s: the instance range exceeds the instance buffer", ctx.shaderName);
    TRHIP_REQUIRE(!ctx.indirect, "%s: dispatched directly", ctx.shaderName);
    const uint64_t threads = (uint64_t)ctx.gx * kNumThreadsPerWave;
    const uint32_t n = threads < k->m_NumInstances ? (uint32_t)threads : k->m_NumInstances;
    if (n == 0) return TRHIP_OK;
    const NodeLocalTransform* np = (const NodeLocalTransform*)nodes->ptr;
    const uint32_t numNodes = (uint32_t)(nodes->byteSize / sizeof(NodeLocalTransform));
    const uint32_t* pn = (const uint32_t*)primToNode->ptr;
    BasePassInstanceConstants* ip = (BasePassInstanceConstants*)instances->ptr;
    ctx.emit("main", [=](hipStream_t s) {
        const uint64_t now = instances->version;
        const trhip::Stamp was = instances->cullCache.built;
        const bool refresh = was.other && was.version + 1 == now && !getenv("TRHIP_NO_CACHE_REFRESH");
        const InstanceCullCache cache = refresh ? instanceCacheLayout(instances->cullCache.ptr, instances->byteSize / sizeof(BasePassInstanceConstants)) : InstanceCullCache{};
        TRHIP_LAUNCH(updateInstanceConstsKernel, dim3((n + kUpdBlock - 1) / kUpdBlock), dim3(kUpdBlock), 0, s, np, numNodes, pn, ip, first, n, refresh, cache);
        if (refresh) instances->cullCache.markBuilt({ now, was.other, was.otherVersion });
        return trhip::launchStatus("updateInstanceConstsKernel"); });
    return TRHIP_OK;
}

trhip::ShaderRegistrar r0("updateinstanceconsts_CS_UpdateInstanceConstsAndBuildTLAS", recordUpdateInstanceConsts, 0);

}
```

toyrenderer_amd/csrc/trhip_core.cpp:

```cpp
#include "trhip_internal.h"
#include "r11g11b10.hip.h"
#include "material_textures.hip.h"

#include <chrono>
#include <cmath>
#include <cstdlib>

#include <algorithm>
#include <memory>

namespace trhip
{

static thread_local char tl_error[1024] = "";

int fail(int code, const char* fmt, ...)
{
    va_list ap;
    va_start(ap, fmt);
    vsnprintf(tl_error, sizeof tl_error, fmt, ap);
    va_end(ap);
    return code;
}

int hipfail(hipError_t e, const char* what)
{
    return fail(TRHIP_ERR_HIP, "HIP error %d (%s) in %s", (int)e, hipGetErrorString(e), what);
}

struct ShaderEntry { std::string name; RecordFn fn; int variant; };
static std::vector<ShaderEntry>& shaders()
{
    static std::vector<ShaderEntry> s;
    return s;
}

void registerShader(const char* name, RecordFn fn, int variant)
{
    shaders().push_back({ name, fn, variant });
}

static const ShaderEntry* findShader(const char* name)
{
    for (const ShaderEntry& e : shaders())
        if (e.name == name) return &e;
    return nullptr;
}

trhip_buffer_t* DispatchCtx::buffer(uint32_t type, uint32_t slot) const
{
    for (uint32_t i = 0; i < numBindings; ++i)
        if (bindings[i].type == type && bindings[i].slot == slot)
            return (trhip_buffer_t*)bindings[i].resource;
    return nullptr;
}

trhip_texture_t* DispatchCtx::texture(uint32_t type, uint32_t slot, uint32_t* baseMip) const
{
    for (uint32_t i = 0; i < numBindings; ++i)
        if (bindings[i].type == type && bindings[i].slot == slot) {
            if (baseMip) *baseMip = bindings[i].baseMip;
            return (trhip_texture_t*)bindings[i].resource;
        }
    return nullptr;
}

trhip_texture_table_t* DispatchCtx::textureTable(uint32_t slot) const
{
    for (uint32_t i = 0; i < numBindings; ++i)
        if (bindings[i].type == TRHIP_BIND_TEXTURE_TABLE && bindings[i].slot == slot)
            return (trhip_texture_table_t*)bindings[i].resource;
    return nullptr;
}

const void* DispatchCtx::constants(uint32_t slot, size_t bytes) const
{
    for (uint32_t i = 0; i < numBindings; ++i) {
        if (bindings[i].slot != slot) continue;
        if (bindings[i].type == TRHIP_BIND_CONSTANT_BUFFER) {
            trhip_buffer_t* b = (trhip_buffer_t*)bindings[i].resource;
            if (!b || !b->isVolatileConstant || b->shadow.size() < bytes) return nullptr;
            return b->shadow.data();
        }
        if (bindings[i].type == TRHIP_BIND_PUSH_CONSTANTS) {
            if (!push || pushBytes < bytes) return nullptr;
            return push;
        }
    }
    return nullptr;
}

void DispatchCtx::emit(const char* kernelName, std::function<int(hipStream_t)> fn) const
{
    std::string n = std::string(shaderName) + "#" + kernelName;
    cl->ops.push_back({ std::move(n), std::move(fn) });
}

void DispatchCtx::emitSide(const char* kernelName, std::function<int(hipStream_t)> fn, std::initializer_list<Op::Access> touched) const
{
    emit(kernelName, std::move(fn));
    if (!cl->dev->sideStream) return;
    cl->ops.back().lane = 1;
    for (const Op::Access& t : touched) if (t.ptr) cl->ops.back().touched.push_back(t);
}

}

using namespace trhip;

namespace
{
struct HostProfile
{
    bool on = getenv("TRHIP_HOST_PROFILE") != nullptr;
    std::mutex m;
    std::map<std::string, std::pair<uint64_t, double>> acc;
    void add(const char* kind, double us)
    {
        std::lock_guard<std::mutex> lk(m);
        auto& e = acc[kind];
        e.first++; e.second += us;
    }
    ~HostProfile()
    {
        if (!on) return;
        for (auto& kv : acc)
            fprintf(stderr, "[trhip host profile] %-14s calls %8llu  total %10.1f us  avg %6.2f us\n", kv.first.c_str(),
                    (unsigned long long)kv.second.first, kv.second.second, kv.second.second / (double)kv.second.first);
    }
} g_hostProfile;
}

thread_local trhip::LaunchTap* trhip::g_launchTap = nullptr;

hipEvent_t trhip_device_t::acquireEvent()
{
    if (!eventPool.empty()) { hipEvent_t e = eventPool.back(); eventPool.pop_back(); return e; }
    hipEvent_t e = nullptr;
    (void)hipEventCreate(&e);
    return e;
}

int trhip_device_t::drainProfile()
{
    for (ProfilePending& p : pending) {
        float ms = 0;
        TRHIP_HIP(hipEventSynchronize(p.e1));
        TRHIP_HIP(hipEventElapsedTime(&ms, p.e0, p.e1));
        auto it = accum.find(p.name);
        if (it == accum.end()) { accumOrder.push_back(p.name); it = accum.emplace(p.name, ProfileAccum{}).first; }
        it->second.launches += 1;
        it->second.totalMs += ms;
        eventPool.push_back(p.e0);
        eventPool.push_back(p.e1);
    }
    pending.clear();
    return TRHIP_OK;
}

static void* arenaAlloc(std::vector<trhip_cmdlist_t::ScratchBlock>& arena, int deviceIndex, size_t bytes)
{
    bytes = (bytes + 255) & ~size_t(255);
    if (bytes == 0) bytes = 256;
    for (trhip_cmdlist_t::ScratchBlock& b : arena)
        if (b.bytes - b.used >= bytes) { void* p = (char*)b.ptr + b.used; b.used += bytes; return p; }
    size_t blockBytes = std::max(bytes, size_t(1) << 20);
    void* p = nullptr;
    if (hipSetDevice(deviceIndex) != hipSuccess || hipMalloc(&p, blockBytes) != hipSuccess) return nullptr;
    arena.push_back({ p, blockBytes, bytes });
    return p;
}

void* trhip_cmdlist_t::scratchAlloc(size_t bytes) { return arenaAlloc(scratch, dev->index, bytes); }
void* trhip_cmdlist_t::scratchAllocSide(size_t bytes) { return arenaAlloc(sideScratch, dev->index, bytes); }

int trhip_device_t::syncAll()
{
    TRHIP_HIP(hipStreamSynchronize(stream));
    if (sideStream) TRHIP_HIP(hipStreamSynchronize(sideStream));
    return TRHIP_OK;
}

int trhip::DerivedData::allocate(const trhip_device_t* dev, uint64_t size)
{
    if (ptr) return size <= bytes ? TRHIP_OK : fail(TRHIP_ERR_STATE, "derived data of %llu bytes asked to grow to %llu", (unsigned long long)bytes, (unsigned long long)size);
    TRHIP_HIP(hipSetDevice(dev->index));
    void* p = nullptr;
    TRHIP_HIP(hipMalloc(&p, (size_t)size));
    ptr = p;
    bytes = size;
    return TRHIP_OK;
}

void trhip::freeDerived(trhip_device_t* dev, std::initializer_list<DerivedData*> all)
{
    bool any = false;
    for (const DerivedData* d : all) any |= d->ptr != nullptr;
    if (!any) return;
    (void)hipSetDevice(dev->index);
    (void)dev->syncAll();
    for (const DerivedData* d : all)
        if (d->ptr) (void)hipFree(d->ptr);
}

void trhip_cmdlist_t::resetRecording()
{
    ops.clear();
    for (trhip_buffer_t* b : heldBuffers) trhip_buffer_release(b);
    for (trhip_texture_t* t : heldTextures) trhip_texture_release(t);
    for (trhip_texture_table_t* t : heldTables) trhip_texture_table_release(t);
    heldBuffers.clear();
    heldTextures.clear();
    heldTables.clear();
    markers.clear();
    openStats = nullptr;
    statsHostCS = 0;
    useMarks.clear();
    openClearBatch.reset();
    openClearOp = SIZE_MAX;
    firstClearBatch.reset();
    firstClearOp = SIZE_MAX;
    clearedTo.clear();
    peephole = Peephole();
    for (ScratchBlock& b : scratch) b.used = 0;
    for (ScratchBlock& b : sideScratch) b.used = 0;
}

namespace
{
struct ClearKernelArgs { void* ptr[trhip_cmdlist_t::ClearBatch::kMax]; uint64_t words[trhip_cmdlist_t::ClearBatch::kMax]; uint32_t value[trhip_cmdlist_t::ClearBatch::kMax]; uint32_t count; };

__global__ __launch_bounds__(256) void multiClearKernel(ClearKernelArgs a)
{
    const uint64_t stride = (uint64_t)gridDim.x * 256u;
    for (uint32_t k = 0; k < a.count; ++k) {
        uint32_t* p = (uint32_t*)a.ptr[k];
        const uint32_t v = a.value[k];
        for (uint64_t i = (uint64_t)blockIdx.x * 256u + threadIdx.x; i < a.words[k]; i += stride) p[i] = v;
    }
}
}

int trhip_cmdlist_t::recordClearWords(void* ptr, uint64_t words, uint32_t value, bool fresh)
{
    if (words == 0) return TRHIP_OK;
    if (fresh && firstClearBatch && firstClearBatch->count < ClearBatch::kMax) {
        ClearBatch& f = *firstClearBatch;
        f.ptr[f.count] = ptr; f.words[f.count] = words; f.value[f.count] = value;
        ++f.count;
        return TRHIP_OK;
    }
    if (!(openClearBatch && openClearOp == ops.size() - 1 && openClearBatch->count < ClearBatch::kMax)) {
        openClearBatch = std::make_shared<ClearBatch>();
        std::shared_ptr<ClearBatch> b = openClearBatch;
        const uint32_t cus = dev->computeUnits;
        ops.push_back({ "", [b, cus](hipStream_t s) {
            ClearKernelArgs a;
            uint64_t most = 0;
            a.count = b->count;
            for (uint32_t k = 0; k < b->count; ++k) { a.ptr[k] = b->ptr[k]; a.words[k] = b->words[k]; a.value[k] = b->value[k]; most = std::max(most, b->words[k]); }
            uint64_t grid = (most + 1023u) / 1024u;
            if (grid > (uint64_t)cus * 8u) grid = (uint64_t)cus * 8u;
            if (grid == 0) grid = 1;
            TRHIP_LAUNCH(multiClearKernel, dim3((uint32_t)grid), dim3(256), 0, s, a);
            return trhip::launchStatus("multiClearKernel"); } });
        ops.back().kind = "clear_buffer";
        openClearOp = ops.size() - 1;
        if (!firstClearBatch) { firstClearBatch = openClearBatch; firstClearOp = openClearOp; }
    }
    ClearBatch& b = *openClearBatch;
    b.ptr[b.count] = ptr; b.words[b.count] = words; b.value[b.count] = value;
    ++b.count;
    return TRHIP_OK;
}

void trhip_cmdlist_t::hold(trhip_buffer_t* b, bool write, size_t op) { if (b) { use(b->ptr, op == SIZE_MAX ? ops.size() : op, write, &b->version); trhip_buffer_retain(b); heldBuffers.push_back(b); } }
void trhip_cmdlist_t::hold(trhip_texture_t* t, bool write) { if (t) { use(t->ptr, ops.size(), write, &t->version); trhip_texture_retain(t); heldTextures.push_back(t); } }

extern "C" {

const char* trhip_last_error(void) { return tl_error; }
uint32_t trhip_abi_version(void) { return TRHIP_ABI_VERSION; }
uint32_t trhip_shader_count(void) { return (uint32_t)shaders().size(); }
const char* trhip_shader_name(uint32_t i) { return i < shaders().size() ? shaders()[i].name.c_str() : nullptr; }
int trhip_shader_exists(const char* name) { return name && findShader(name) ? 1 : 0; }

static int deviceCreate(int index, void* stream, bool external, trhip_device* out)
{
    if (!out) return fail(TRHIP_ERR_INVALID, "out is null");
    int n = 0;
    if (hipGetDeviceCount(&n) != hipSuccess || n <= 0)
        return fail(TRHIP_ERR_NO_DEVICE, "no HIP device visible (this back end has no CPU fallback)");
    if (index < 0 || index >= n) return fail(TRHIP_ERR_INVALID, "device index %d out of range (%d devices)", index, n);
    TRHIP_HIP(hipSetDevice(index));
    hipDeviceProp_t props;
    TRHIP_HIP(hipGetDeviceProperties(&props, index));
    auto dev = std::make_unique<trhip_device_t>();
    dev->index = index;
    dev->computeUnits = (uint32_t)props.multiProcessorCount;
    dev->waveSize = (uint32_t)props.warpSize;
    dev->totalMem = (uint64_t)props.totalGlobalMem;
    if (dev->waveSize != 64)
        return fail(TRHIP_ERR_INVALID, "wave size %u: the kernels are written for wave64 (gfx950)", dev->waveSize);
    if (external) {
        dev->stream = (hipStream_t)stream;
        dev->ownsStream = false;
    } else {
        TRHIP_HIP(hipStreamCreateWithFlags(&dev->stream, hipStreamNonBlocking));
        dev->ownsStream = true;
    }
    if (!getenv("TRHIP_NO_SIDE_STREAM")) {
        int lowest = 0, highest = 0;
        TRHIP_HIP(hipDeviceGetStreamPriorityRange(&lowest, &highest));
        TRHIP_HIP(hipStreamCreateWithPriority(&dev->sideStream, hipStreamNonBlocking, highest));
        TRHIP_HIP(hipEventCreateWithFlags(&dev->evFork, hipEventDisableTiming));
        for (hipEvent_t& e : dev->runDone) TRHIP_HIP(hipEventCreateWithFlags(&e, hipEventDisableTiming));
    }
    *out = dev.release();
    return TRHIP_OK;
}

int trhip_device_create(int device_index, trhip_device* out) { return deviceCreate(device_index, nullptr, false, out); }
int trhip_device_create_on_stream(int device_index, void* s, trhip_device* out) { return deviceCreate(device_index, s, true, out); }

void trhip_device_destroy(trhip_device dev)
{
    if (!dev) return;
    (void)hipSetDevice(dev->index);
    (void)dev->syncAll();
    (void)dev->drainProfile();
    for (hipEvent_t e : dev->eventPool) (void)hipEventDestroy(e);
    if (dev->sideStream) { (void)hipStreamSynchronize(dev->sideStream); (void)hipStreamDestroy(dev->sideStream); }
    if (dev->evFork) (void)hipEventDestroy(dev->evFork);
    for (hipEvent_t e : dev->runDone) if (e) (void)hipEventDestroy(e);
    if (dev->srgbTable.ptr) (void)hipFree(dev->srgbTable.ptr);
    if (dev->ownsStream) (void)hipStreamDestroy(dev->stream);
    delete dev;
}

int trhip_device_wait_idle(trhip_device dev)
{
    if (!dev) return fail(TRHIP_ERR_INVALID, "device is null");
    TRHIP_HIP(hipSetDevice(dev->index));
    return dev->syncAll();
}

int trhip_device_join_side_stream(trhip_device dev)
{
    if (!dev) return fail(TRHIP_ERR_INVALID, "device is null");
    TRHIP_HIP(hipSetDevice(dev->index));
    std::lock_guard<std::mutex> lock(dev->mutex);
    if (dev->sideStream && dev->sideRunCounter > dev->mainWaitedUpTo) {
        TRHIP_HIP(hipStreamWaitEvent(dev->stream, dev->runDone[dev->sideRunCounter % trhip_device_t::kSideRuns], 0));
        dev->mainWaitedUpTo = dev->sideRunCounter;
    }
    return TRHIP_OK;
}

int trhip_device_info(trhip_device dev, uint32_t* cus, uint32_t* wave, uint64_t* mem)
{
    if (!dev) return fail(TRHIP_ERR_INVALID, "device is null");
    if (cus) *cus = dev->computeUnits;
    if (wave) *wave = dev->waveSize;
    if (mem) *mem = dev->totalMem;
    return TRHIP_OK;
}

void* trhip_device_stream(trhip_device dev) { return dev ? (void*)dev->stream : nullptr; }

int trhip_heap_create(trhip_device dev, uint64_t bytes, trhip_heap* out)
{
    if (!dev || !out || bytes == 0) return fail(TRHIP_ERR_INVALID, "heap_create: bad arguments");
    TRHIP_HIP(hipSetDevice(dev->index));
    auto h = std::make_unique<trhip_heap_t>();
    h->dev = dev;
    h->bytes = bytes;
    TRHIP_HIP(hipMalloc(&h->base, bytes));
    *out = h.release();
    return TRHIP_OK;
}

static void heapRetain(trhip_heap_t* h) { if (h) h->rc.fetch_add(1); }

void trhip_heap_release(trhip_heap h)
{
    if (!h) return;
    if (h->rc.fetch_sub(1) == 1) {
        (void)hipSetDevice(h->dev->index);
        (void)hipFree(h->base);
        delete h;
    }
}

static void fillBuffer(trhip_buffer_t* b, trhip_device dev, const trhip_buffer_desc* d)
{
    b->dev = dev;
    b->byteSize = d->byteSize;
    b->structStride = d->structStride;
    b->canHaveUAVs = d->canHaveUAVs != 0;
    b->isDrawIndirectArgs = d->isDrawIndirectArgs != 0;
    b->isVirtual = d->isVirtual != 0;
    b->isVolatileConstant = d->isVolatileConstant != 0;
    b->name = d->debugName ? d->debugName : "";
}

int trhip_buffer_create(trhip_device dev, const trhip_buffer_desc* desc, trhip_buffer* out)
{
    if (!dev || !desc || !out) return fail(TRHIP_ERR_INVALID, "buffer_create: null argument");
    if (desc->byteSize == 0) return fail(TRHIP_ERR_INVALID, "buffer_create(%s): byteSize is 0", desc->debugName ? desc->debugName : "");
    auto b = std::make_unique<trhip_buffer_t>();
    fillBuffer(b.get(), dev, desc);
    if (b->isVolatileConstant) {
        b->shadow.assign((size_t)desc->byteSize, 0);
    } else if (!b->isVirtual) {
        TRHIP_HIP(hipSetDevice(dev->index));
        TRHIP_HIP(hipMalloc(&b->ptr, (size_t)((desc->byteSize + 255) & ~uint64_t(255))));
        b->owns = true;
    }
    *out = b.release();
    return TRHIP_OK;
}

int trhip_buffer_wrap(trhip_device dev, void* ptr, const trhip_buffer_desc* desc, trhip_buffer* out)
{
    if (!dev || !desc || !out || !ptr) return fail(TRHIP_ERR_INVALID, "buffer_wrap: null argument");
    if (desc->byteSize == 0) return fail(TRHIP_ERR_INVALID, "buffer_wrap: byteSize is 0");
    auto b = std::make_unique<trhip_buffer_t>();
    fillBuffer(b.get(), dev, desc);
    b->isVirtual = false;
    b->ptr = ptr;
    b->owns = false;
    *out = b.release();
    return TRHIP_OK;
}

int trhip_buffer_memory_requirements(trhip_buffer buf, uint64_t* size, uint64_t* alignment)
{
    if (!buf) return fail(TRHIP_ERR_INVALID, "buffer is null");
    if (size) *size = (buf->byteSize + 255) & ~uint64_t(255);
    if (alignment) *alignment = 256;
    return TRHIP_OK;
}

int trhip_buffer_bind_memory(trhip_buffer buf, trhip_heap heap, uint64_t offset)
{
    if (!buf || !heap) return fail(TRHIP_ERR_INVALID, "bind_memory: null argument");
    if (!buf->isVirtual) return fail(TRHIP_ERR_STATE, "bind_memory(%s): buffer is not virtual", buf->name.c_str());
    if (offset % 256) return fail(TRHIP_ERR_INVALID, "bind_memory(%s): offset %llu not 256-byte aligned", buf->name.c_str(), (unsigned long long)offset);
    if (offset + buf->byteSize > heap->bytes) return fail(TRHIP_ERR_INVALID, "bind_memory(%s): range exceeds the heap", buf->name.c_str());
    if (buf->heap) trhip_heap_release(buf->heap);
    heapRetain(heap);
    buf->heap = heap;
    buf->ptr = (char*)heap->base + offset;
    buf->version.fetch_add(1);
    return TRHIP_OK;
}

void trhip_buffer_retain(trhip_buffer b) { if (b) b->rc.fetch_add(1); }

void trhip_buffer_release(trhip_buffer b)
{
    if (!b) return;
    if (b->rc.fetch_sub(1) == 1) {
        if (b->owns && b->ptr) { (void)hipSetDevice(b->dev->index); (void)hipFree(b->ptr); }
        trhip::freeDerived(b->dev, { &b->cullCache, &b->cullStream, &b->triCounts, &b->order, &b->listCount });
        if (b->heap) trhip_heap_release(b->heap);
        delete b;
    }
}

void* trhip_buffer_device_ptr(trhip_buffer b) { return b ? b->ptr : nullptr; }
uint64_t trhip_buffer_size(trhip_buffer b) { return b ? b->byteSize : 0; }

static int createTexture(trhip_device dev, const trhip_texture_desc* d, uint32_t arraySize, trhip_texture* out)
{
    if (d->width == 0 || d->height == 0 || d->mipLevels == 0 || d->mipLevels > 16)
        return fail(TRHIP_ERR_INVALID, "texture_create: bad dimensions %ux%u mips %u", d->width, d->height, d->mipLevels);
    if ((d->format < TRHIP_FORMAT_R16_FLOAT || d->format > TRHIP_FORMAT_R8_UINT) && (d->format < TRHIP_FORMAT_RGBA8_UNORM || d->format > TRHIP_FORMAT_RGBA16_FLOAT))
        return fail(TRHIP_ERR_INVALID, "texture_create: unsupported format %u", d->format);
    const bool bloomChain = d->format == TRHIP_FORMAT_R11G11B10_FLOAT && (d->isUAV & TRHIP_TEXTURE_RENDER_TARGET);
    const bool sampledChain = (d->format == TRHIP_FORMAT_RGBA8_UNORM || d->format == TRHIP_FORMAT_SRGBA8_UNORM) && d->isUAV == 0;
    if (d->format != TRHIP_FORMAT_R16_FLOAT && d->format != TRHIP_FORMAT_R32_FLOAT && !bloomChain && !sampledChain && d->mipLevels != 1)
        return fail(TRHIP_ERR_INVALID, "texture_create: RG32_UINT / RG16_FLOAT / RGBA32_UINT / R11G11B10_FLOAT / R8_UNORM / R8_UINT / R10G10B10A2_UNORM / RGBA16_FLOAT textures and RGBA8_UNORM / SRGBA8_UNORM textures that a pass writes have one mip, got %u", d->mipLevels);
    if (arraySize) {
        if (arraySize > 2048) return fail(TRHIP_ERR_INVALID, "texture_create_array: %u slices, at most 2048", arraySize);
        if (d->format != TRHIP_FORMAT_R10G10B10A2_UNORM && d->format != TRHIP_FORMAT_RG16_FLOAT && d->format != TRHIP_FORMAT_RGBA16_FLOAT)
            return fail(TRHIP_ERR_INVALID, "texture_create_array: format %u; an array texture is R10G10B10A2_UNORM, RG16_FLOAT or RGBA16_FLOAT", d->format);
        if (d->mipLevels != 1) return fail(TRHIP_ERR_INVALID, "texture_create_array: an array texture has one mip, got %u", d->mipLevels);
    }
    auto t = std::make_unique<trhip_texture_t>();
    t->dev = dev;
    t->width = d->width; t->height = d->height; t->mips = d->mipLevels; t->format = d->format;
    t->texelBytes = d->format == TRHIP_FORMAT_R16_FLOAT ? 2 : d->format == TRHIP_FORMAT_RG32_UINT || d->format == TRHIP_FORMAT_RGBA16_FLOAT ? 8 :
                    d->format == TRHIP_FORMAT_RGBA32_UINT ? 16 : d->format == TRHIP_FORMAT_R8_UNORM || d->format == TRHIP_FORMAT_R8_UINT ? 1 : 4;
    t->isUAV = d->isUAV != 0; t->isVirtual = d->isVirtual != 0;
    t->name = d->debugName ? d->debugName : "";
    uint64_t off = 0;
    for (uint32_t k = 0; k < t->mips; ++k) {
        t->mipOffset[k] = off;
        off += ((uint64_t)t->mipW(k) * t->mipH(k) * t->texelBytes + 255) & ~uint64_t(255);
    }
    if (arraySize) {
        t->arraySize = arraySize;
        t->slicePitch = off;
        off *= arraySize;
    }
    t->totalBytes = off;
    if (!t->isVirtual) {
        TRHIP_HIP(hipSetDevice(dev->index));
        TRHIP_HIP(hipMalloc(&t->ptr, (size_t)off));
        t->owns = true;
    }
    *out = t.release();
    return TRHIP_OK;
}

int trhip_texture_create(trhip_device dev, const trhip_texture_desc* d, trhip_texture* out)
{
    if (!dev || !d || !out) return fail(TRHIP_ERR_INVALID, "texture_create: null argument");
    return createTexture(dev, d, 0, out);
}

int trhip_texture_create_array(trhip_device dev, const trhip_texture_desc* d, uint32_t arraySize, trhip_texture* out)
{
    if (!dev || !d || !out) return fail(TRHIP_ERR_INVALID, "texture_create_array: null argument");
    if (arraySize == 0) return fail(TRHIP_ERR_INVALID, "texture_create_array: an array texture has at least one slice");
    return createTexture(dev, d, arraySize, out);
}

uint32_t trhip_texture_array_size(trhip_texture t) { return t ? t->arraySize : 0; }
uint64_t trhip_texture_slice_pitch(trhip_texture t) { return t ? t->slicePitch : 0; }

int trhip_texture_memory_requirements(trhip_texture t, uint64_t* size, uint64_t* alignment)
{
    if (!t) return fail(TRHIP_ERR_INVALID, "texture is null");
    if (size) *size = t->totalBytes;
    if (alignment) *alignment = 256;
    return TRHIP_OK;
}

int trhip_texture_bind_memory(trhip_texture t, trhip_heap heap, uint64_t offset)
{
    if (!t || !heap) return fail(TRHIP_ERR_INVALID, "bind_memory: null argument");
    if (!t->isVirtual) return fail(TRHIP_ERR_STATE, "bind_memory(%s): texture is not virtual", t->name.c_str());
    if (offset % 256 || offset + t->totalBytes > heap->bytes) return fail(TRHIP_ERR_INVALID, "bind_memory(%s): bad range", t->name.c_str());
    if (t->heap) trhip_heap_release(t->heap);
    heapRetain(heap);
    t->heap = heap;
    t->ptr = (char*)heap->base + offset;
    t->version.fetch_add(1);
    return TRHIP_OK;
}

void trhip_texture_retain(trhip_texture t) { if (t) t->rc.fetch_add(1); }

void trhip_texture_release(trhip_texture t)
{
    if (!t) return;
    if (t->rc.fetch_sub(1) == 1) {
        if (t->owns && t->ptr) { (void)hipSetDevice(t->dev->index); (void)hipFree(t->ptr); }
        trhip::freeDerived(t->dev, { &t->quad });
        if (t->heap) trhip_heap_release(t->heap);
        delete t;
    }
}

void* trhip_texture_device_ptr(trhip_texture t) { return t ? t->ptr : nullptr; }
uint64_t trhip_texture_size(trhip_texture t) { return t ? t->totalBytes : 0; }

int trhip_texture_mip_info(trhip_texture t, uint32_t mip, uint32_t* w, uint32_t* h, uint64_t* off)
{
    if (!t || mip >= t->mips) return fail(TRHIP_ERR_INVALID, "mip_info: bad texture/mip");
    if (w) *w = t->mipW(mip);
    if (h) *h = t->mipH(mip);
    if (off) *off = t->mipOffset[mip];
    return TRHIP_OK;
}

static int syncCopy(trhip_device_t* dev, void* dst, const void* src, uint64_t bytes, hipMemcpyKind kind)
{
    TRHIP_HIP(hipSetDevice(dev->index));
    int rc = dev->syncAll();
    if (rc != TRHIP_OK) return rc;
    TRHIP_HIP(hipMemcpy(dst, src, (size_t)bytes, kind));
    return TRHIP_OK;
}

int trhip_buffer_upload(trhip_buffer b, uint64_t off, const void* src, uint64_t bytes)
{
    if (!b || !src) return fail(TRHIP_ERR_INVALID, "buffer_upload: null argument");
    if (!b->ptr) return fail(TRHIP_ERR_STATE, "buffer_upload(%s): no memory bound", b->name.c_str());
    if (off + bytes > b->byteSize) return fail(TRHIP_ERR_INVALID, "buffer_upload(%s): range exceeds the buffer", b->name.c_str());
    int rc = syncCopy(b->dev, (char*)b->ptr + off, src, bytes, hipMemcpyHostToDevice);
    b->version.fetch_add(1);
    return rc;
}

int trhip_buffer_mark_written(trhip_buffer b)
{
    if (!b) return fail(TRHIP_ERR_INVALID, "buffer_mark_written: null argument");
    b->version.fetch_add(1);
    return TRHIP_OK;
}

int trhip_texture_mark_written(trhip_texture t)
{
    if (!t) return fail(TRHIP_ERR_INVALID, "texture_mark_written: null argument");
    t->version.fetch_add(1);
    return TRHIP_OK;
}

int trhip_buffer_download(trhip_buffer b, uint64_t off, void* dst, uint64_t bytes)
{
    if (!b || !dst) return fail(TRHIP_ERR_INVALID, "buffer_download: null argument");
    if (!b->ptr) return fail(TRHIP_ERR_STATE, "buffer_download(%s): no memory bound", b->name.c_str());
    if (off + bytes > b->byteSize) return fail(TRHIP_ERR_INVALID, "buffer_download(%s): range exceeds the buffer", b->name.c_str());
    return syncCopy(b->dev, dst, (char*)b->ptr + off, bytes, hipMemcpyDeviceToHost);
}

int trhip_texture_upload(trhip_texture t, uint32_t mip, const void* src, uint64_t bytes)
{
    if (!t || !src || mip >= t->mips) return fail(TRHIP_ERR_INVALID, "texture_upload: bad argument");
    if (!t->ptr) return fail(TRHIP_ERR_STATE, "texture_upload(%s): no memory bound", t->name.c_str());
    if (t->arraySize) return fail(TRHIP_ERR_INVALID, "texture_upload(%s): an array texture is uploaded per slice (trhip_texture_upload_slice)", t->name.c_str());
    uint64_t need = (uint64_t)t->mipW(mip) * t->mipH(mip) * t->texelBytes;
    if (bytes != need) return fail(TRHIP_ERR_INVALID, "texture_upload(%s): mip %u is %llu bytes, got %llu", t->name.c_str(), mip, (unsigned long long)need, (unsigned long long)bytes);
    int rc = syncCopy(t->dev, t->mipPtr(mip), src, bytes, hipMemcpyHostToDevice);
    t->version.fetch_add(1);
    return rc;
}

int trhip_texture_download(trhip_texture t, uint32_t mip, void* dst, uint64_t bytes)
{
    if (!t || !dst || mip >= t->mips) return fail(TRHIP_ERR_INVALID, "texture_download: bad argument");
    if (!t->ptr) return fail(TRHIP_ERR_STATE, "texture_download(%s): no memory bound", t->name.c_str());
    if (t->arraySize) return fail(TRHIP_ERR_INVALID, "texture_download(%s): an array texture is downloaded per slice (trhip_texture_download_slice)", t->name.c_str());
    uint64_t need = (uint64_t)t->mipW(mip) * t->mipH(mip) * t->texelBytes;
    if (bytes != need) return fail(TRHIP_ERR_INVALID, "texture_download(%s): mip %u is %llu bytes, got %llu", t->name.c_str(), mip, (unsigned long long)need, (unsigned long long)bytes);
    return syncCopy(t->dev, dst, t->mipPtr(mip), bytes, hipMemcpyDeviceToHost);
}

static int sliceRange(trhip_texture t, uint32_t slice, uint64_t bytes, const char* what)
{
    if (!t->arraySize) return fail(TRHIP_ERR_INVALID, "%s(%s): not an array texture", what, t->name.c_str());
    if (slice >= t->arraySize) return fail(TRHIP_ERR_INVALID, "%s(%s): slice %u, the texture has %u", what, t->name.c_str(), slice, t->arraySize);
    if (!t->ptr) return fail(TRHIP_ERR_STATE, "%s(%s): no memory bound", what, t->name.c_str());
    const uint64_t need = (uint64_t)t->width * t->height * t->texelBytes;
    if (bytes != need) return fail(TRHIP_ERR_INVALID, "%s(%s): a slice is %llu bytes, got %llu", what, t->name.c_str(), (unsigned long long)need, (unsigned long long)bytes);
    return TRHIP_OK;
}

int trhip_texture_upload_slice(trhip_texture t, uint32_t slice, const void* src, uint64_t bytes)
{
    if (!t || !src) return fail(TRHIP_ERR_INVALID, "texture_upload_slice: null argument");
    if (const int rc = sliceRange(t, slice, bytes, "texture_upload_slice")) return rc;
    const int rc = syncCopy(t->dev, (char*)t->ptr + slice * t->slicePitch, src, bytes, hipMemcpyHostToDevice);
    t->version.fetch_add(1);
    return rc;
}

int trhip_texture_download_slice(trhip_texture t, uint32_t slice, void* dst, uint64_t bytes)
{
    if (!t || !dst) return fail(TRHIP_ERR_INVALID, "texture_download_slice: null argument");
    if (const int rc = sliceRange(t, slice, bytes, "texture_download_slice")) return rc;
    return syncCopy(t->dev, dst, (char*)t->ptr + slice * t->slicePitch, bytes, hipMemcpyDeviceToHost);
}

int trhip_srgb_table(float* out)
{
    if (!out) return fail(TRHIP_ERR_INVALID, "srgb_table: out is null");
    for (int i = 0; i < 256; ++i) {
        const double c = (double)i / 255.0;
        out[i] = (float)(c <= 0.04045 ? c / 12.92 : std::pow((c + 0.055) / 1.055, 2.4));
    }
    return TRHIP_OK;
}

int trhip_texture_table_create(trhip_device dev, uint32_t capacity, trhip_texture_table* out)
{
    if (!dev || !out) return fail(TRHIP_ERR_INVALID, "texture_table_create: null argument");
    if (capacity == 0 || capacity > (1u << 20)) return fail(TRHIP_ERR_INVALID, "texture_table_create: capacity %u not in 1 .. 2^20", capacity);
    TRHIP_HIP(hipSetDevice(dev->index));
    {
        std::lock_guard<std::mutex> lock(dev->mutex);
        if (!dev->srgbTable.ptr) {
            float table[256];
            trhip_srgb_table(table);
            trhip::DerivedData filled;
            int rc = filled.allocate(dev, sizeof table);
            if (rc != TRHIP_OK) return rc;
            hipError_t e = hipMemcpy(filled.ptr, table, sizeof table, hipMemcpyHostToDevice);
            if (e != hipSuccess) { (void)hipFree(filled.ptr); return hipfail(e, "hipMemcpy(sRGB table)"); }
            dev->srgbTable = filled;
        }
    }
    auto t = std::make_unique<trhip_texture_table_t>();
    t->dev = dev;
    t->slots.assign(capacity, nullptr);
    int rc = t->entries.allocate(dev, (uint64_t)capacity * sizeof(mtex::TableEntry));
    if (rc != TRHIP_OK) return rc;
    hipError_t e = hipMemset(t->entries.ptr, 0, (size_t)t->entries.bytes);
    if (e != hipSuccess) { (void)hipFree(t->entries.ptr); return hipfail(e, "hipMemset(texture table)"); }
    *out = t.release();
    return TRHIP_OK;
}

void trhip_texture_table_retain(trhip_texture_table t) { if (t) t->rc.fetch_add(1); }

void trhip_texture_table_release(trhip_texture_table t)
{
    if (!t) return;
    if (t->rc.fetch_sub(1) == 1) {
        trhip::freeDerived(t->dev, { &t->entries });
        for (trhip_texture_t* e : t->slots) trhip_texture_release(e);
        delete t;
    }
}

uint32_t trhip_texture_table_capacity(trhip_texture_table t) { return t ? (uint32_t)t->slots.size() : 0; }

static int tableWrite(trhip_texture_table_t* t, uint32_t index, trhip_texture_t* tex)
{
    mtex::TableEntry e;
    memset(&e, 0, sizeof e);
    if (tex) {
        e.base = (const uint32_t*)tex->ptr;
        e.width = tex->width; e.height = tex->height; e.mips = tex->mips; e.format = tex->format;
        for (uint32_t k = 0; k < tex->mips; ++k) e.mipOffset[k] = (uint32_t)(tex->mipOffset[k] / 4u);
    }
    int rc = syncCopy(t->dev, (char*)t->entries.ptr + (uint64_t)index * sizeof e, &e, sizeof e, hipMemcpyHostToDevice);
    if (rc != TRHIP_OK) return rc;
    trhip_texture_retain(tex);
    trhip_texture_release(t->slots[index]);
    t->slots[index] = tex;
    return TRHIP_OK;
}

int trhip_texture_table_set(trhip_texture_table t, uint32_t index, trhip_texture tex)
{
    if (!t || !tex) return fail(TRHIP_ERR_INVALID, "texture_table_set: null argument");
    if (index >= t->slots.size()) return fail(TRHIP_ERR_INVALID, "texture_table_set: index %u at or past the capacity %zu", index, t->slots.size());
    if (tex->dev != t->dev) return fail(TRHIP_ERR_INVALID, "texture_table_set(%s): the texture belongs to another device", tex->name.c_str());
    if (!tex->ptr) return fail(TRHIP_ERR_STATE, "texture_table_set(%s): no memory bound", tex->name.c_str());
    if (tex->totalBytes / 4u > 0xFFFFFFFFull) return fail(TRHIP_ERR_INVALID, "texture_table_set(%s): more than 2^32 texels", tex->name.c_str());
    if (tex->arraySize) return fail(TRHIP_ERR_INVALID, "texture_table_set(%s): an array texture cannot be a table entry", tex->name.c_str());
    return tableWrite(t, index, tex);
}

int trhip_texture_table_clear(trhip_texture_table t, uint32_t index)
{
    if (!t) return fail(TRHIP_ERR_INVALID, "texture_table_clear: null argument");
    if (index >= t->slots.size()) return fail(TRHIP_ERR_INVALID, "texture_table_clear: index %u at or past the capacity %zu", index, t->slots.size());
    return tableWrite(t, index, nullptr);
}
// ... 218 lines not shown
}

static int recordDispatch(trhip_cmdlist cl, const char* name, const trhip_binding* b, uint32_t nb, const void* push, uint32_t pushBytes,
                          bool indirect, trhip_buffer args, uint32_t argsOff, uint32_t gx, uint32_t gy, uint32_t gz)
{
    TRHIP_RECORDING(cl);
    if (!name) return fail(TRHIP_ERR_INVALID, "dispatch: shader name is null");
    const ShaderEntry* e = findShader(name);
    if (!e) return fail(TRHIP_ERR_UNKNOWN_SHADER, "dispatch: unknown shader '%s'", name);
    if (nb && !b) return fail(TRHIP_ERR_INVALID, "dispatch(%s): bindings is null", name);
    if (indirect) {
        if (!args || !args->ptr) return fail(TRHIP_ERR_INVALID, "dispatch_indirect(%s): no argument buffer", name);
        if (argsOff % 4 || argsOff + 12 > args->byteSize) return fail(TRHIP_ERR_INVALID, "dispatch_indirect(%s): bad argument offset %u", name, argsOff);
        cl->hold(args, false);
    } else if (gx == 0 || gy == 0 || gz == 0) {
        return fail(TRHIP_ERR_INVALID, "dispatch(%s): zero group count (Graphic.cpp:944)", name);
    }
    for (uint32_t i = 0; i < nb; ++i) {
        switch (b[i].type) {
        case TRHIP_BIND_CONSTANT_BUFFER: case TRHIP_BIND_STRUCTURED_SRV: case TRHIP_BIND_STRUCTURED_UAV: {
            trhip_buffer_t* r = (trhip_buffer_t*)b[i].resource;
            if (!r) return fail(TRHIP_ERR_INVALID, "dispatch(%s): binding %u has no buffer", name, i);
            if (b[i].type != TRHIP_BIND_CONSTANT_BUFFER && !r->ptr) return fail(TRHIP_ERR_STATE, "dispatch(%s): buffer '%s' has no memory bound", name, r->name.c_str());
            if (b[i].type == TRHIP_BIND_STRUCTURED_UAV && !r->canHaveUAVs) return fail(TRHIP_ERR_INVALID, "dispatch(%s): buffer '%s' bound as UAV without canHaveUAVs", name, r->name.c_str());
            cl->hold(r, b[i].type == TRHIP_BIND_STRUCTURED_UAV);
            break; }
        case TRHIP_BIND_TEXTURE_SRV: case TRHIP_BIND_TEXTURE_UAV: {
            trhip_texture_t* t = (trhip_texture_t*)b[i].resource;
            if (!t) return fail(TRHIP_ERR_INVALID, "dispatch(%s): binding %u has no texture", name, i);
            if (!t->ptr) return fail(TRHIP_ERR_STATE, "dispatch(%s): texture '%s' has no memory bound", name, t->name.c_str());
            if (b[i].type == TRHIP_BIND_TEXTURE_UAV && b[i].baseMip >= t->mips) return fail(TRHIP_ERR_INVALID, "dispatch(%s): UAV mip %u out of range", name, b[i].baseMip);
            if (t->arraySize)
                if (const int rc = checkArrayBinding(name, b[i], t)) return rc;
            cl->hold(t, b[i].type == TRHIP_BIND_TEXTURE_UAV);
            break; }
        case TRHIP_BIND_TEXTURE_TABLE: {
            trhip_texture_table_t* t = (trhip_texture_table_t*)b[i].resource;
            if (!t) return fail(TRHIP_ERR_INVALID, "dispatch(%s): binding %u has no texture table", name, i);
            if (t->dev != cl->dev) return fail(TRHIP_ERR_INVALID, "dispatch(%s): the texture table belongs to another device", name);
            static const char* const kTableShaders[] = { "basepass_PS_Main_GBuffer", "basepass_MS_Main_depth ALPHA_MASK_MODE=1", "basepass_MS_Main_visibility ALPHA_MASK_MODE=1",
                                                         "shadowmask_CS_ShadowMask" };
            bool declares = false;
            for (const char* n : kTableShaders) declares |= strcmp(name, n) == 0;
            if (!declares || b[i].slot != 19u)
                return fail(TRHIP_ERR_INVALID, "dispatch(%s): a texture table at t%u: only basepass_PS_Main_GBuffer, the ALPHA_MASK_MODE=1 rasters and shadowmask_CS_ShadowMask declare one, at t19",
                            name, b[i].slot);
            trhip_texture_table_retain(t);
            cl->heldTables.push_back(t);
            for (trhip_texture_t* e : t->slots) cl->hold(e, false);
            break; }
        case TRHIP_BIND_PUSH_CONSTANTS: case TRHIP_BIND_SAMPLER: break;
        default: return fail(TRHIP_ERR_INVALID, "dispatch(%s): binding %u has unknown type %u", name, i, b[i].type);
        }
    }
    DispatchCtx ctx{ cl, e->name.c_str(), e->variant, b, nb, push, pushBytes, indirect, args, argsOff, gx, gy, gz };
    int rc = e->fn(ctx);
    if (rc != TRHIP_OK || !cl->openStats) return rc;
    const uint32_t threads = statsCSThreads(name);
    if (!threads) return TRHIP_OK;
    if (!indirect) { cl->statsHostCS += (uint64_t)gx * gy * gz * threads; return TRHIP_OK; }
    return statsEmitIndirectCS(cl, args, argsOff, threads);
}

int trhip_cmd_dispatch(trhip_cmdlist cl, const char* name, const trhip_binding* b, uint32_t nb, const void* push, uint32_t pushBytes,
                       uint32_t gx, uint32_t gy, uint32_t gz)
{
    return recordDispatch(cl, name, b, nb, push, pushBytes, false, nullptr, 0, gx, gy, gz);
}

int trhip_cmd_dispatch_indirect(trhip_cmdlist cl, const char* name, const trhip_binding* b, uint32_t nb, const void* push, uint32_t pushBytes,
                                trhip_buffer args, uint32_t argsOff)
{
    return recordDispatch(cl, name, b, nb, push, pushBytes, true, args, argsOff, 0, 0, 0);
}

int trhip_cmd_begin_timer(trhip_cmdlist cl, trhip_timer t)
{
    TRHIP_RECORDING(cl);
    if (!t) return fail(TRHIP_ERR_INVALID, "timer is null");
    cl->ops.push_back({ "", [t](hipStream_t s) { TRHIP_HIP(hipEventRecord(t->e0, s)); t->began = true; t->ended = false; return (int)TRHIP_OK; } });
    cl->ops.back().kind = "timer";
    return TRHIP_OK;
}

int trhip_cmd_end_timer(trhip_cmdlist cl, trhip_timer t)
{
    TRHIP_RECORDING(cl);
    if (!t) return fail(TRHIP_ERR_INVALID, "timer is null");
    cl->ops.push_back({ "", [t](hipStream_t s) { TRHIP_HIP(hipEventRecord(t->e1, s)); t->ended = true; return (int)TRHIP_OK; } });
    cl->ops.back().kind = "timer";
    return TRHIP_OK;
}

int trhip_cmd_begin_pipeline_stats(trhip_cmdlist cl, trhip_pipeline_stats q)
{
    TRHIP_RECORDING(cl);
    if (!q) return fail(TRHIP_ERR_INVALID, "pipeline statistics query is null");
    if (q->dev != cl->dev) return fail(TRHIP_ERR_INVALID, "begin_pipeline_stats: the query belongs to another device");
    if (cl->openStats) return fail(TRHIP_ERR_STATE, "begin_pipeline_stats: this command list already has a query open");
    cl->openStats = q;
    cl->statsHostCS = 0;
    cl->peephole = trhip_cmdlist_t::Peephole();
    cl->use(q->counters, cl->ops.size(), true);
    cl->ops.push_back({ "", [q](hipStream_t s) {
        TRHIP_HIP(hipMemsetAsync(q->counters, 0, sizeof(trhip_pipeline_statistics), s));
        q->began = true; q->ended = false;
        return (int)TRHIP_OK; } });
    cl->ops.back().kind = "pipeline_stats";
    return TRHIP_OK;
}

int trhip_cmd_end_pipeline_stats(trhip_cmdlist cl, trhip_pipeline_stats q)
{
    TRHIP_RECORDING(cl);
    if (!q) return fail(TRHIP_ERR_INVALID, "pipeline statistics query is null");
    if (cl->openStats != q) return fail(TRHIP_ERR_STATE, "end_pipeline_stats: the query is not open in this command list");
    const uint64_t hostCS = cl->statsHostCS;
    cl->openStats = nullptr;
    cl->statsHostCS = 0;
    cl->peephole = trhip_cmdlist_t::Peephole();
    cl->use(q->counters, cl->ops.size(), true);
    cl->ops.push_back({ "", [q, hostCS](hipStream_t s) {
        if (hostCS) {
            int rc = statsLaunchAdd(q->counters + kStatCS, hostCS, s);
            if (rc != TRHIP_OK) return rc;
        }
        TRHIP_HIP(hipEventRecord(q->done, s));
        q->ended = true;
        return (int)TRHIP_OK; } });
    cl->ops.back().kind = "pipeline_stats";
    return TRHIP_OK;
}

int trhip_cmd_begin_marker(trhip_cmdlist cl, const char* name)
{
    TRHIP_RECORDING(cl);
    cl->markers.push_back(name ? name : "");
    return TRHIP_OK;
}

int trhip_cmd_end_marker(trhip_cmdlist cl)
{
    TRHIP_RECORDING(cl);
    if (cl->markers.empty()) return fail(TRHIP_ERR_STATE, "end_marker without begin_marker");
    cl->markers.pop_back();
    return TRHIP_OK;
}

int trhip_queue_execute(trhip_device dev, const trhip_cmdlist* lists, uint32_t n)
{
    if (!dev || (n && !lists)) return fail(TRHIP_ERR_INVALID, "queue_execute: null argument");
    TRHIP_HIP(hipSetDevice(dev->index));
    std::lock_guard<std::mutex> lock(dev->mutex);
    bool inRun = false;
    std::vector<Op::Access> runTouched;
    auto endRun = [&]() -> int {
        if (!inRun) return TRHIP_OK;
        inRun = false;
        const uint64_t id = ++dev->sideRunCounter;
        const uint32_t slot = (uint32_t)(id % trhip_device_t::kSideRuns);
        if (id > trhip_device_t::kSideRuns && id - trhip_device_t::kSideRuns > dev->mainWaitedUpTo) {
            TRHIP_HIP(hipStreamWaitEvent(dev->stream, dev->runDone[slot], 0));
            dev->mainWaitedUpTo = id - trhip_device_t::kSideRuns;
        }
        TRHIP_HIP(hipEventRecord(dev->runDone[slot], dev->sideStream));
        for (const Op::Access& t : runTouched) (t.write ? dev->sideWriter : dev->sideReader)[t.ptr] = id;
        runTouched.clear();
        return TRHIP_OK;
    };
    auto ownerOf = [&](const void* ptr, bool write) -> uint64_t {
        uint64_t need = 0;
        auto w = dev->sideWriter.find(ptr);
        if (w != dev->sideWriter.end()) need = w->second;
        if (write) {
            auto r = dev->sideReader.find(ptr);
            if (r != dev->sideReader.end() && r->second > need) need = r->second;
        }
        return need;
    };
    auto waitForRun = [&](uint64_t need) -> int {
        if (need <= dev->mainWaitedUpTo) return TRHIP_OK;
        TRHIP_HIP(hipStreamWaitEvent(dev->stream, dev->runDone[need % trhip_device_t::kSideRuns], 0));
        dev->mainWaitedUpTo = need;
        return TRHIP_OK;
    };
    auto nextIsSide = [&](uint32_t li, size_t oi) -> bool {
        if (!dev->sideStream) return false;
        for (++oi; li < n; ++li, oi = 0)
            if (lists[li] && oi < lists[li]->ops.size()) return lists[li]->ops[oi].lane == 1;
        return false;
    };
    for (uint32_t i = 0; i < n; ++i) {
        trhip_cmdlist_t* cl = lists[i];
        if (!cl) return fail(TRHIP_ERR_INVALID, "queue_execute: list %u is null", i);
        if (cl->open) return fail(TRHIP_ERR_STATE, "queue_execute: list %u is still open", i);
        if (cl->dev != dev) return fail(TRHIP_ERR_INVALID, "queue_execute: list %u belongs to another device", i);
        size_t mark = 0;
        for (size_t oi = 0; oi < cl->ops.size(); ++oi) {
            const Op& op = cl->ops[oi];
            const bool side = op.lane == 1 && dev->sideStream;
            hipStream_t stream = dev->stream;
            if (side) {
                if (!inRun) {
                    if (!dev->forkSignalled) TRHIP_HIP(hipEventRecord(dev->evFork, dev->stream));
                    dev->forkSignalled = false;
                    TRHIP_HIP(hipStreamWaitEvent(dev->sideStream, dev->evFork, 0));
                    inRun = true;
                }
                runTouched.insert(runTouched.end(), op.touched.begin(), op.touched.end());
                stream = dev->sideStream;
                for (; mark < cl->useMarks.size() && cl->useMarks[mark].op <= oi; ++mark)
                    if (cl->useMarks[mark].write && cl->useMarks[mark].version) cl->useMarks[mark].version->fetch_add(1);
            } else {
                int rc = endRun();
                if (rc != TRHIP_OK) return rc;
                uint64_t need = 0;
                for (; mark < cl->useMarks.size() && cl->useMarks[mark].op <= oi; ++mark) {
                    const trhip_cmdlist_t::UseMark& m = cl->useMarks[mark];
                    need = std::max(need, ownerOf(m.ptr, m.write));
                    if (m.write && m.version) m.version->fetch_add(1);
                }
                rc = waitForRun(need);
                if (rc != TRHIP_OK) return rc;
            }
            const bool prof = dev->profiling && !op.name.empty() && (dev->profileFilter.empty() || dev->profileFilter == op.name);
            hipEvent_t e0 = nullptr, e1 = nullptr;
            if (prof) { e0 = dev->acquireEvent(); e1 = dev->acquireEvent(); TRHIP_HIP(hipEventRecord(e0, stream)); }
            const auto h0 = g_hostProfile.on ? std::chrono::steady_clock::now() : std::chrono::steady_clock::time_point{};
            trhip::LaunchTap tap;
            dev->forkSignalled = false;
            const bool tapped = !side && !prof && strcmp(op.kind, "host_callback") != 0 && nextIsSide(i, oi);
            if (tapped) { tap.onStream = stream; tap.stopEvent = dev->evFork; trhip::g_launchTap = &tap; }
            int rc = op.fn(stream);
            trhip::g_launchTap = nullptr;
            if (tapped && tap.launches >= 1 && rc == TRHIP_OK) dev->forkSignalled = true;
            if (g_hostProfile.on) g_hostProfile.add(op.kind, std::chrono::duration<double, std::micro>(std::chrono::steady_clock::now() - h0).count());
            if (rc != TRHIP_OK) return rc;
            if (prof) { TRHIP_HIP(hipEventRecord(e1, stream)); dev->pending.push_back({ op.name, e0, e1 }); }
        }
    }
    return endRun();
}

int trhip_stream_create_priority(int device_index, int priority_class, void** out)
{
    if (!out) return fail(TRHIP_ERR_INVALID, "stream_create: out is null");
    TRHIP_HIP(hipSetDevice(device_index));
    int lowest = 0, highest = 0;
    TRHIP_HIP(hipDeviceGetStreamPriorityRange(&lowest, &highest));
    hipStream_t s = nullptr;
    TRHIP_HIP(hipStreamCreateWithPriority(&s, hipStreamNonBlocking, priority_class < 0 ? highest : priority_class > 0 ? lowest : 0));
    *out = (void*)s;
    return TRHIP_OK;
}

int trhip_stream_create(int device_index, void** out) { return trhip_stream_create_priority(device_index, 0, out); }

void trhip_stream_destroy(void* s)
{
    if (s) { (void)hipStreamSynchronize((hipStream_t)s); (void)hipStreamDestroy((hipStream_t)s); }
}

int trhip_stream_synchronize(void* s)
{
    TRHIP_HIP(hipStreamSynchronize((hipStream_t)s));
    return TRHIP_OK;
}

int trhip_event_create(int device_index, void** out)
{
    if (!out) return fail(TRHIP_ERR_INVALID, "event_create: out is null");
    TRHIP_HIP(hipSetDevice(device_index));
    hipEvent_t e = nullptr;
    TRHIP_HIP(hipEventCreateWithFlags(&e, hipEventDisableTiming));
    *out = (void*)e;
    return TRHIP_OK;
}

void trhip_event_destroy(void* e)
{
    if (e) (void)hipEventDestroy((hipEvent_t)e);
}

int trhip_event_record(void* e, void* s)
{
    if (!e) return fail(TRHIP_ERR_INVALID, "event_record: event is null");
    TRHIP_HIP(hipEventRecord((hipEvent_t)e, (hipStream_t)s));
    return TRHIP_OK;
}

int trhip_stream_wait_event(void* s, void* e)
{
    if (!e) return fail(TRHIP_ERR_INVALID, "stream_wait_event: event is null");
    TRHIP_HIP(hipStreamWaitEvent((hipStream_t)s, (hipEvent_t)e, 0));
    return TRHIP_OK;
}

int trhip_timer_create(trhip_device dev, trhip_timer* out)
{
    if (!dev || !out) return fail(TRHIP_ERR_INVALID, "timer_create: null argument");
    TRHIP_HIP(hipSetDevice(dev->index));
    auto t = std::make_unique<trhip_timer_t>();
    t->dev = dev;
    TRHIP_HIP(hipEventCreate(&t->e0));
    TRHIP_HIP(hipEventCreate(&t->e1));
    *out = t.release();
    return TRHIP_OK;
}

void trhip_timer_release(trhip_timer t)
{
    if (!t) return;
    (void)hipEventDestroy(t->e0);
    (void)hipEventDestroy(t->e1);
    delete t;
}

int trhip_timer_get_ms(trhip_timer t, float* ms)
{
    if (!t || !ms) return fail(TRHIP_ERR_INVALID, "timer_get_ms: null argument");
    if (!t->began || !t->ended) return fail(TRHIP_ERR_STATE, "timer_get_ms: timer was not begun and ended in an executed list");
    TRHIP_HIP(hipEventSynchronize(t->e1));
    TRHIP_HIP(hipEventElapsedTime(ms, t->e0, t->e1));
    return TRHIP_OK;
}

int trhip_pipeline_stats_create(trhip_device dev, trhip_pipeline_stats* out)
{
    if (!dev || !out) return fail(TRHIP_ERR_INVALID, "pipeline_stats_create: null argument");
    TRHIP_HIP(hipSetDevice(dev->index));
    auto q = std::make_unique<trhip_pipeline_stats_t>();
    q->dev = dev;
    TRHIP_HIP(hipMalloc(&q->counters, sizeof(trhip_pipeline_statistics)));
    TRHIP_HIP(hipMemset(q->counters, 0, sizeof(trhip_pipeline_statistics)));
    TRHIP_HIP(hipEventCreateWithFlags(&q->done, hipEventDisableTiming));
    *out = q.release();
    return TRHIP_OK;
}

void trhip_pipeline_stats_release(trhip_pipeline_stats q)
{
    if (!q) return;
    (void)hipSetDevice(q->dev->index);
    (void)q->dev->syncAll();
    (void)hipFree(q->counters);
    (void)hipEventDestroy(q->done);
    delete q;
}

int trhip_pipeline_stats_get(trhip_pipeline_stats q, trhip_pipeline_statistics* out)
{
    if (!q || !out) return fail(TRHIP_ERR_INVALID, "pipeline_stats_get: null argument");
    if (!q->began || !q->ended) return fail(TRHIP_ERR_STATE, "pipeline_stats_get: query was not begun and ended in an executed list");
    TRHIP_HIP(hipSetDevice(q->dev->index));
    TRHIP_HIP(hipEventSynchronize(q->done));
    TRHIP_HIP(hipMemcpy(out, q->counters, sizeof(trhip_pipeline_statistics), hipMemcpyDeviceToHost));
    return TRHIP_OK;
}

int trhip_profile_enable(trhip_device dev, int enabled)
{
    if (!dev) return fail(TRHIP_ERR_INVALID, "device is null");
    std::lock_guard<std::mutex> lock(dev->mutex);
    dev->profiling = enabled != 0;
    return TRHIP_OK;
}

int trhip_profile_filter(trhip_device dev, const char* name)
{
    if (!dev) return fail(TRHIP_ERR_INVALID, "device is null");
    std::lock_guard<std::mutex> lock(dev->mutex);
    dev->profileFilter = name ? name : "";
    return TRHIP_OK;
}

int trhip_profile_reset(trhip_device dev)
{
    if (!dev) return fail(TRHIP_ERR_INVALID, "device is null");
    std::lock_guard<std::mutex> lock(dev->mutex);
    int rc = dev->drainProfile();
    dev->accum.clear();
    dev->accumOrder.clear();
    return rc;
}

int trhip_profile_count(trhip_device dev, uint32_t* n)
{
    if (!dev || !n) return fail(TRHIP_ERR_INVALID, "profile_count: null argument");
    std::lock_guard<std::mutex> lock(dev->mutex);
    int rc = dev->drainProfile();
    *n = (uint32_t)dev->accumOrder.size();
    return rc;
}

// ... 15 lines not shown
```

toyrenderer_amd/csrc/trhip_internal.h:

```cpp
#pragma once

#include <hip/hip_runtime.h>

#include <atomic>
#include <cstdarg>
#include <cstdint>
#include <cstdio>
#include <cstdlib>
#include <cstring>
#include <functional>
#include <map>
#include <memory>
#include <mutex>
#include <string>
#include <unordered_map>
#include <vector>

#include <hip/hip_ext.h>

#include "../../include/trhip.h"
#include "ShaderInterop.h"

namespace trhip
{

int fail(int code, const char* fmt, ...) __attribute__((format(printf, 2, 3)));
int hipfail(hipError_t e, const char* what);

#define TRHIP_HIP(expr)                                                        \
    do {                                                                       \
        hipError_t _e = (expr);                                                \
        if (_e != hipSuccess) return ::trhip::hipfail(_e, #expr);              \
    } while (0)

#define TRHIP_REQUIRE(cond, ...)                                               \
    do {                                                                       \
        if (!(cond)) return ::trhip::fail(TRHIP_ERR_INVALID, __VA_ARGS__);     \
    } while (0)

struct ProfilePending { std::string name; hipEvent_t e0, e1; };
struct ProfileAccum { uint64_t launches = 0; double totalMs = 0; };

}

struct trhip_device_t;

namespace trhip
{

struct Stamp
{
    uint64_t version = 0;
    const void* other = nullptr;
    uint64_t otherVersion = 0;
    bool operator==(const Stamp& s) const { return version == s.version && other == s.other && otherVersion == s.otherVersion; }
};

struct DerivedData
{
    void* ptr = nullptr;
    uint64_t bytes = 0;
    Stamp built;

    int allocate(const trhip_device_t* dev, uint64_t size);
    bool current(const Stamp& s) const { return built == s; }
    void markBuilt(const Stamp& s) { built = s; }
};

}

struct trhip_device_t
{
    int index = 0;
    hipStream_t stream = nullptr;
    bool ownsStream = false;
    uint32_t computeUnits = 0;
    uint32_t waveSize = 0;
    uint64_t totalMem = 0;

    static constexpr uint32_t kSideRuns = 16;
    hipStream_t sideStream = nullptr;
    hipEvent_t evFork = nullptr;
    bool forkSignalled = false;
    hipEvent_t runDone[kSideRuns] = {};
    uint64_t sideRunCounter = 0;
    uint64_t mainWaitedUpTo = 0;
    std::unordered_map<const void*, uint64_t> sideWriter;
    std::unordered_map<const void*, uint64_t> sideReader;
    int syncAll();

    std::mutex mutex;
    bool profiling = false;
    std::string profileFilter;
    std::vector<trhip::ProfilePending> pending;
    std::vector<hipEvent_t> eventPool;
    std::map<std::string, trhip::ProfileAccum> accum;
    std::vector<std::string> accumOrder;

    hipEvent_t acquireEvent();
    int drainProfile();

    trhip::DerivedData srgbTable;
};

struct trhip_heap_t
{
    trhip_device_t* dev = nullptr;
    void* base = nullptr;
    uint64_t bytes = 0;
    std::atomic<int> rc{1};
};

namespace trhip
{

void freeDerived(trhip_device_t* dev, std::initializer_list<DerivedData*> all);

}

struct trhip_buffer_t
{
    trhip_device_t* dev = nullptr;
    uint64_t byteSize = 0;
    uint32_t structStride = 0;
    bool canHaveUAVs = false, isDrawIndirectArgs = false, isVirtual = false, isVolatileConstant = false;
    std::string name;
    void* ptr = nullptr;
    bool owns = false;
    trhip_heap_t* heap = nullptr;
    std::vector<uint8_t> shadow;
    std::atomic<uint64_t> version{1};
    trhip::DerivedData cullCache;
    trhip::DerivedData cullStream;
    trhip::DerivedData triCounts;
    trhip::DerivedData order;
    trhip::DerivedData listCount;
    std::atomic<int> rc{1};
};

struct trhip_texture_t
{
    trhip_device_t* dev = nullptr;
    uint32_t width = 0, height = 0, mips = 0, format = 0;
    uint32_t texelBytes = 0;
    bool isUAV = false, isVirtual = false;
    uint32_t arraySize = 0;
    uint64_t slicePitch = 0;
    std::string name;
    uint64_t mipOffset[16] = {};
    uint64_t totalBytes = 0;
    void* ptr = nullptr;
    bool owns = false;
    trhip_heap_t* heap = nullptr;
    trhip::DerivedData quad;
    uint32_t quadOffset[16] = {};
    uint32_t quadTotal = 0;
    std::atomic<uint64_t> version{1};
    std::atomic<int> rc{1};

    uint32_t mipW(uint32_t k) const { return (width >> k) ? (width >> k) : 1u; }
    uint32_t mipH(uint32_t k) const { return (height >> k) ? (height >> k) : 1u; }
    void* mipPtr(uint32_t k) const { return (char*)ptr + mipOffset[k]; }
};

struct trhip_texture_table_t
{
    trhip_device_t* dev = nullptr;
    std::vector<trhip_texture_t*> slots;
    trhip::DerivedData entries;
    std::atomic<int> rc{1};
};

struct trhip_timer_t
{
    trhip_device_t* dev = nullptr;
    hipEvent_t e0 = nullptr, e1 = nullptr;
    bool began = false, ended = false;
};

struct MeshletCullArgs;

struct trhip_pipeline_stats_t
{
    trhip_device_t* dev = nullptr;
    unsigned long long* counters = nullptr;
    hipEvent_t done = nullptr;
    bool began = false, ended = false;
};

namespace trhip
{

enum : uint32_t { kStatCS = 10, kStatAS = 11, kStatMS = 12, kStatMSPrim = 13, kStatWords = 14 };

struct Op
{
    std::string name;
    std::function<int(hipStream_t)> fn;
    const char* kind = "dispatch";
    uint8_t lane = 0;
    struct Access { const void* ptr; bool write; };
    std::vector<Access> touched;
};

}

struct trhip_cmdlist_t
{
    trhip_device_t* dev = nullptr;
    bool open = false;
    std::vector<trhip::Op> ops;
    std::vector<trhip_buffer_t*> heldBuffers;
    std::vector<trhip_texture_t*> heldTextures;
    std::vector<trhip_texture_table_t*> heldTables;
    std::vector<std::string> markers;
    trhip_pipeline_stats_t* openStats = nullptr;
    uint64_t statsHostCS = 0;

    struct ScratchBlock { void* ptr; size_t bytes; size_t used; };
    std::vector<ScratchBlock> scratch;

    struct ClearBatch { static constexpr uint32_t kMax = 32; void* ptr[kMax]; uint64_t words[kMax]; uint32_t value[kMax]; uint32_t count = 0; };
    std::shared_ptr<ClearBatch> openClearBatch;
    size_t openClearOp = SIZE_MAX;
    std::shared_ptr<ClearBatch> firstClearBatch;
    size_t firstClearOp = SIZE_MAX;
    struct ClearedTo { uint32_t value; size_t marks; };
    std::unordered_map<const void*, ClearedTo> clearedTo;
    bool stillClearedTo(const void* ptr, uint32_t value) const
    {
        auto it = clearedTo.find(ptr);
        if (it == clearedTo.end() || it->second.value != value) return false;
        for (size_t i = it->second.marks; i < useMarks.size(); ++i)
            if (useMarks[i].ptr == ptr && useMarks[i].write) return false;
        return true;
    }
    int recordClearWords(void* ptr, uint64_t words, uint32_t value, bool fresh = false);
    bool usedSoFar(const void* ptr) const { for (const UseMark& m : useMarks) if (m.ptr == ptr) return true; return false; }

    struct UseMark { size_t op; const void* ptr; bool write; std::atomic<uint64_t>* version; };
    std::vector<UseMark> useMarks;
    void use(const void* ptr, size_t op, bool write, std::atomic<uint64_t>* version = nullptr)
    {
        if (!ptr) return;
        useMarks.push_back({ op, ptr, write, version });
    }
    void forgetUse(const void* ptr, size_t op)
    {
        for (size_t i = useMarks.size(); i-- > 0 && useMarks[i].op >= op;)
            if (useMarks[i].op == op && useMarks[i].ptr == ptr) useMarks.erase(useMarks.begin() + (ptrdiff_t)i);
    }

    struct Peephole { size_t op = SIZE_MAX; const char* kind = nullptr; std::shared_ptr<void> data; } peephole;

    void* scratchAlloc(size_t bytes);
    void* scratchAllocSide(size_t bytes);
    std::vector<ScratchBlock> sideScratch;
    void resetRecording();
    void hold(trhip_buffer_t* b, bool write, size_t op = SIZE_MAX);
    void hold(trhip_texture_t* t, bool write);
};

namespace trhip
{

struct DispatchCtx
{
    trhip_cmdlist_t* cl;
    const char* shaderName;
    int variant;
    const trhip_binding* bindings; uint32_t numBindings;
    const void* push; uint32_t pushBytes;
    bool indirect; trhip_buffer_t* argsBuffer; uint32_t argsOffset;
    uint32_t gx, gy, gz;

    trhip_buffer_t* buffer(uint32_t type, uint32_t slot) const;
    trhip_texture_t* texture(uint32_t type, uint32_t slot, uint32_t* baseMip = nullptr) const;
    trhip_texture_table_t* textureTable(uint32_t slot) const;
    const void* constants(uint32_t slot, size_t bytes) const;
    uint32_t computeUnits() const { return cl->dev->computeUnits; }
    void* scratch(size_t bytes) const { return cl->scratchAlloc(bytes); }
    void* scratchSide(size_t bytes) const { return cl->dev->sideStream ? cl->scratchAllocSide(bytes) : cl->scratchAlloc(bytes); }
    void emit(const char* kernelName, std::function<int(hipStream_t)> fn) const;
    void emitSide(const char* kernelName, std::function<int(hipStream_t)> fn, std::initializer_list<Op::Access> touched) const;
};

int hzbQuadEnsure(trhip_texture_t* tex);
int hzbQuadLaunchBuild(trhip_texture_t* tex, hipStream_t s);

int instanceCacheEnsure(trhip_buffer_t* instances);
int instanceCacheLaunchBuild(trhip_buffer_t* instances, trhip_buffer_t* meshData, hipStream_t s);

inline uint32_t tableMinGroups()
{
    static const uint32_t v = [] { const char* e = getenv("TRHIP_TABLE_MIN_GROUPS"); return e ? (uint32_t)strtoul(e, nullptr, 0) : (1u << 17); }();
    return v;
}

uint32_t statsCSThreads(const char* shaderName);
int statsLaunchAdd(unsigned long long* counter, uint64_t value, hipStream_t s);
int statsEmitIndirectCS(trhip_cmdlist_t* cl, trhip_buffer_t* args, uint32_t argsOffset, uint32_t threads);
int statsEmitAS(const DispatchCtx& ctx, const ::MeshletCullArgs& a, trhip_buffer_t* meshlets, trhip_buffer_t* records,
                trhip_buffer_t* instances, trhip_buffer_t* meshData, bool side);

using RecordFn = int (*)(DispatchCtx&);
void registerShader(const char* name, RecordFn fn, int variant);

struct ShaderRegistrar
{
    ShaderRegistrar(const char* name, RecordFn fn, int variant = 0) { registerShader(name, fn, variant); }
};

struct LaunchTap { hipStream_t onStream = nullptr; hipEvent_t stopEvent = nullptr; int launches = 0; };
extern thread_local LaunchTap* g_launchTap;
#define TRHIP_LAUNCH(kernel, grid, block, shmem, stream, ...)                                                       \
    do {                                                                                                            \
        trhip::LaunchTap* tap_ = trhip::g_launchTap;                                                                \
        if (tap_ && tap_->onStream == (stream) && ++tap_->launches)                                              \
            hipExtLaunchKernelGGL(kernel, grid, block, shmem, stream, nullptr, tap_->stopEvent, 0, __VA_ARGS__);    \
        else                                                                                                        \
            hipLaunchKernelGGL(kernel, grid, block, shmem, stream, __VA_ARGS__);                                    \
    } while (0)

inline int launchStatus(const char* what)
{
    hipError_t e = hipGetLastError();
    return e == hipSuccess ? TRHIP_OK : hipfail(e, what);
}

}
```

Measured before the change: 120.0.

## Run instance transform update on a low-priority ahead stream with double-buffered cache

Adds a third low-priority "ahead" stream that runs the instance-update kernel ahead of the main stream. The transform part of the instance cull cache is double-buffered (live/spare), so next-frame updates can overlap culling that still reads the current generation. Cull kernels now resolve the live generation at launch time, and the dependency tracking is generalised to per-lane maps, fork events and generation-aware use marks. The cost is an extra device-to-device copy when the update range changes, plus considerably more complex cross-stream synchronisation that could serialise or race.

```diff
diff --git a/toyrenderer_amd/csrc/host/nvrhi_lite.h b/toyrenderer_amd/csrc/host/nvrhi_lite.h
--- a/toyrenderer_amd/csrc/host/nvrhi_lite.h
+++ b/toyrenderer_amd/csrc/host/nvrhi_lite.h
@@ -492,6 +492,7 @@
         throwIfFailed(trhip_device_join_side_stream(producer), "IDevice::queueWaitForCommandList: join");
         throwIfFailed(trhip_event_record(ev, trhip_device_stream(producer)), "IDevice::queueWaitForCommandList: record");
         throwIfFailed(trhip_stream_wait_event(trhip_device_stream(queueDevice(waitQueue)), ev), "IDevice::queueWaitForCommandList: wait");
+        throwIfFailed(trhip_device_join_side_stream(queueDevice(waitQueue)), "IDevice::queueWaitForCommandList: join (waiting queue)");
     }
     uint64_t lastInstance(CommandQueue queue) const { return m_LastInstance[(size_t)queue]; }
     bool hasComputeQueue() const { return m_ComputeNative != nullptr; }
diff --git a/toyrenderer_amd/csrc/instance_cache.hip.h b/toyrenderer_amd/csrc/instance_cache.hip.h
--- a/toyrenderer_amd/csrc/instance_cache.hip.h
+++ b/toyrenderer_amd/csrc/instance_cache.hip.h
@@ -21,13 +21,17 @@
 
 constexpr uint64_t kInstanceCacheBytesPerInstance = 64 + 16 + 4 + 4 + 3 * 4 * interop::kMaxNumMeshLODs + 16;
 
-inline InstanceCullCache instanceCacheLayout(void* base, uint64_t n)
+constexpr uint64_t kInstanceCacheTransformBytesPerInstance = 64 + 16 + 4;
+
+inline InstanceCullCache instanceCacheLayout(void* base, uint64_t n, void* transform = nullptr)
 {
     char* p = (char*)base;
+    char* t = transform ? (char*)transform : p;
     InstanceCullCache c;
-    c.world = (const float4*)p;             p += 64 * n;
-    c.sphere = (const float4*)p;            p += 16 * n;
-    c.maxScale = (const float*)p;           p += 4 * n;
+    c.world = (const float4*)t;             t += 64 * n;
+    c.sphere = (const float4*)t;            t += 16 * n;
+    c.maxScale = (const float*)t;
+    p += kInstanceCacheTransformBytesPerInstance * n;
     c.numLODs = (const uint32_t*)p;         p += 4 * n;
     c.lodInfo = (const uint2*)p;            p += 8ull * interop::kMaxNumMeshLODs * n;
     c.error = (const float*)p;              p += 4ull * interop::kMaxNumMeshLODs * n;
diff --git a/toyrenderer_amd/csrc/k_basepass_as.hip b/toyrenderer_amd/csrc/k_basepass_as.hip
--- a/toyrenderer_amd/csrc/k_basepass_as.hip
+++ b/toyrenderer_amd/csrc/k_basepass_as.hip
@@ -1277,6 +1277,8 @@
     if (rc != TRHIP_OK) return rc;
     a.numInstances = (uint32_t)(instances->byteSize / sizeof(BasePassInstanceConstants));
     a.cache = instanceCacheLayout(instances->cullCache.ptr, a.numInstances);
+    ctx.cl->forgetUse(instances->ptr, ctx.cl->ops.size());
+    trhip::instanceCacheUse(ctx.cl, instances);
     a.maxBatches = (a.recordCapacity + kBatch - 1) / kBatch;
     a.batchSum = (uint32_t*)(a.recordCapacity >= (1u << 19) ? ctx.scratchSide((size_t)a.maxBatches * 4)
                                                             : ctx.scratch((size_t)a.maxBatches * 4));
@@ -1303,7 +1305,9 @@
     trhip_texture_t* quadOwner = useTable ? hzb : nullptr;
     const bool table = useTable;
     if (quadOwner) ctx.cl->use(quadOwner->quad.ptr, ctx.cl->ops.size(), false);
-    ctx.emit("cull", [a, grid, flags, quadOwner, table, instances, meshData, meshlets](hipStream_t s) {
+    ctx.emit("cull", [a0 = a, grid, flags, quadOwner, table, instances, meshData, meshlets](hipStream_t s) {
+        MeshletCullArgs a = a0;
+        a.cache = instanceCacheLayout(instances->cullCache.ptr, a.numInstances, instances->cullCache.live());
         if ((const void*)a.meshlets != meshlets->ptr)
             return trhip::fail(TRHIP_ERR_STATE, "basepass_AS_Main: the meshlet buffer was bound to other memory after this command list was recorded: record it again");
         {
diff --git a/toyrenderer_amd/csrc/k_gpuculling.hip b/toyrenderer_amd/csrc/k_gpuculling.hip
--- a/toyrenderer_amd/csrc/k_gpuculling.hip
+++ b/toyrenderer_amd/csrc/k_gpuculling.hip
@@ -47,7 +47,14 @@
     uint32_t* lateArgsOut;
     unsigned long long* fusedStatus;
     uint32_t* fusedTicket;
+    trhip_buffer_t* cacheOwner;
 };
+
+inline InstanceCullArgs liveCache(InstanceCullArgs a)
+{
+    if (a.cacheOwner) a.cache = instanceCacheLayout(a.cacheOwner->cullCache.ptr, a.numInstances, a.cacheOwner->cullCache.live());
+    return a;
+}
 
 struct QuadShare { bool stale = false; };
 struct EarlyCullNote { InstanceCullArgs a; size_t scanOp; bool fused; trhip_texture_t* quadOwner = nullptr; std::shared_ptr<QuadShare> share; };
@@ -623,7 +630,7 @@
             strips = q.firstStrip[q.mips];
             quadOwner->quad.markBuilt({ quadOwner->version });
         }
-        TRHIP_LAUNCH(instanceFusedKernel<0>, dim3(a.numBlocks + strips), dim3(kBlock), 0, s, a, q);
+        TRHIP_LAUNCH(instanceFusedKernel<0>, dim3(a.numBlocks + strips), dim3(kBlock), 0, s, liveCache(a), q);
         return trhip::launchStatus("instanceFusedKernel"); };
 }
 
@@ -647,7 +654,7 @@
             quadOwner->quad.markBuilt({ quadOwner->version });
             if (share) share->stale = true;
         }
-        TRHIP_LAUNCH(instanceScanKernel<0>, dim3(1 + kScanTileGroups + extra), dim3(kScanThreads), 0, s, a, q, stripEnd);
+        TRHIP_LAUNCH(instanceScanKernel<0>, dim3(1 + kScanTileGroups + extra), dim3(kScanThreads), 0, s, liveCache(a), q, stripEnd);
         return trhip::launchStatus("instanceScanKernel"); };
 }
 
@@ -712,6 +719,9 @@
     if (rc != TRHIP_OK) return rc;
     a.cache = instanceCacheLayout(instances->cullCache.ptr, instances->byteSize / sizeof(BasePassInstanceConstants));
     a.numInstances = (uint32_t)(instances->byteSize / sizeof(BasePassInstanceConstants));
+    a.cacheOwner = instances;
+    ctx.cl->forgetUse(instances->ptr, ctx.cl->ops.size());
+    trhip::instanceCacheUse(ctx.cl, instances);
     ctx.emit("instance_cache", [instances, meshData](hipStream_t s) { return trhip::instanceCacheLaunchBuild(instances, meshData, s); });
     static const bool noFused = getenv("TRHIP_NO_FUSED_INSTANCE") != nullptr;
     const bool fusedPath = (nMax <= kFusedMaxEntries || (LATE && (nMax + kBlock - 1) / kBlock <= kFusedLateMaxTiles)) && !noFused;
@@ -747,30 +757,34 @@
         a.fusedTicket = mem + (size_t)a.numBlocks * kFusedStatusStride * 2;
         trhip_texture_t* quadOwner = wantTable ? hzb : nullptr;
         if (quadOwner) ctx.cl->use(quadOwner->quad.ptr, ctx.cl->ops.size(), true);
+        trhip::instanceCacheUse(ctx.cl, instances);
         if (LATE) ctx.emit("fused", [a](hipStream_t s) {
             trhip::QuadArgs q;
             memset(&q, 0, sizeof q);
-            TRHIP_LAUNCH(instanceFusedKernel<LATE>, dim3(a.numBlocks), dim3(kBlock), 0, s, a, q);
+            TRHIP_LAUNCH(instanceFusedKernel<LATE>, dim3(a.numBlocks), dim3(kBlock), 0, s, liveCache(a), q);
             return trhip::launchStatus("instanceFusedKernel"); });
         else ctx.emit("fused", fusedEarlyLaunch(a, quadOwner));
         if (!LATE && occlusion) ctx.cl->peephole = { ctx.cl->ops.size() - 1, "gpuculling_early", std::make_shared<EarlyCullNote>(EarlyCullNote{ a, ctx.cl->ops.size() - 1, true, quadOwner }) };
         return TRHIP_OK;
     }
 
+    trhip::instanceCacheUse(ctx.cl, instances);
     ctx.emit("classify", [a](hipStream_t s) {
-        TRHIP_LAUNCH(instanceClassifyKernel<LATE>, dim3(a.numBlocks), dim3(kBigThreads), 0, s, a);
+        TRHIP_LAUNCH(instanceClassifyKernel<LATE>, dim3(a.numBlocks), dim3(kBigThreads), 0, s, liveCache(a));
         return trhip::launchStatus("instanceClassifyKernel"); });
     trhip_texture_t* quadOwner = wantTable ? hzb : nullptr;
     std::shared_ptr<QuadShare> share = quadOwner ? std::make_shared<QuadShare>() : nullptr;
     if (quadOwner) ctx.cl->use(quadOwner->quad.ptr, ctx.cl->ops.size(), true);
+    trhip::instanceCacheUse(ctx.cl, instances);
     if (LATE) ctx.emit("scan", [a](hipStream_t s) {
         trhip::QuadArgs q;
         memset(&q, 0, sizeof q);
-        TRHIP_LAUNCH(instanceScanKernel<LATE>, dim3(1 + kScanTileGroups), dim3(kScanThreads), 0, s, a, q, 0u);
+        TRHIP_LAUNCH(instanceScanKernel<LATE>, dim3(1 + kScanTileGroups), dim3(kScanThreads), 0, s, liveCache(a), q, 0u);
         return trhip::launchStatus("instanceScanKernel"); });
     else ctx.emit("scan", scanEarlyLaunch(a, quadOwner, share));
     const size_t scanOp = ctx.cl->ops.size() - 1;
     if (quadOwner) ctx.cl->use(quadOwner->quad.ptr, ctx.cl->ops.size(), true);
+    trhip::instanceCacheUse(ctx.cl, instances);
     ctx.emit("emit", [a, quadOwner, share](hipStream_t s) {
         trhip::QuadArgs q;
         memset(&q, 0, sizeof q);
@@ -780,7 +794,7 @@
             stripBegin = quadScanStrips(q.firstStrip[q.mips]);
             extra = (q.firstStrip[q.mips] - stripBegin + kEmitStripsPerGroup - 1u) / kEmitStripsPerGroup;
         }
-        TRHIP_LAUNCH(instanceEmitKernel<LATE>, dim3(a.numBlocks + extra), dim3(kBigThreads), 0, s, a, q, stripBegin);
+        TRHIP_LAUNCH(instanceEmitKernel<LATE>, dim3(a.numBlocks + extra), dim3(kBigThreads), 0, s, liveCache(a), q, stripBegin);
         return trhip::launchStatus("instanceEmitKernel"); });
     if (!LATE && occlusion) ctx.cl->peephole = { ctx.cl->ops.size() - 1, "gpuculling_early", std::make_shared<EarlyCullNote>(EarlyCullNote{ a, scanOp, false, quadOwner, share }) };
     return TRHIP_OK;
@@ -831,15 +845,22 @@
     return instances->cullCache.allocate(instances->dev, n * kInstanceCacheBytesPerInstance);
 }
 
+void instanceCacheUse(trhip_cmdlist_t* cl, trhip_buffer_t* instances)
+{
+    cl->use(instances->cullCache.ptr, cl->ops.size(), false, nullptr, &instances->cullCache);
+}
+
 int instanceCacheLaunchBuild(trhip_buffer_t* instances, trhip_buffer_t* meshData, hipStream_t s)
 {
     const Stamp from = { instances->version, meshData->ptr, meshData->version };
     if (instances->cullCache.current(from)) return TRHIP_OK;
     const uint32_t n = (uint32_t)(instances->byteSize / sizeof(BasePassInstanceConstants));
     const uint64_t numMeshes = meshData->byteSize / sizeof(MeshData);
+    if (const int rc = instances->dev->joinAhead(s)) return rc;
+    instances->cullGenLevel.level = false;
     TRHIP_LAUNCH(instanceCacheKernel, dim3((n + 255u) / 256u), dim3(256), 0, s, (const BasePassInstanceConstants*)instances->ptr, n,
                        (const MeshData*)meshData->ptr, (uint32_t)(numMeshes > 0xFFFFFFFFull ? 0xFFFFFFFFull : numMeshes),
-                       instanceCacheLayout(instances->cullCache.ptr, n));
+                       instanceCacheLayout(instances->cullCache.ptr, n, instances->cullCache.live()));
     instances->cullCache.markBuilt(from);
     return launchStatus("instanceCacheKernel");
 }
diff --git a/toyrenderer_amd/csrc/k_updateinstance.hip b/toyrenderer_amd/csrc/k_updateinstance.hip
--- a/toyrenderer_amd/csrc/k_updateinstance.hip
+++ b/toyrenderer_amd/csrc/k_updateinstance.hip
@@ -147,14 +147,34 @@
     const uint32_t numNodes = (uint32_t)(nodes->byteSize / sizeof(NodeLocalTransform));
     const uint32_t* pn = (const uint32_t*)primToNode->ptr;
     BasePassInstanceConstants* ip = (BasePassInstanceConstants*)instances->ptr;
-    ctx.emit("main", [=](hipStream_t s) {
+    const uint64_t numRecords = instances->byteSize / sizeof(BasePassInstanceConstants);
+    int rc = trhip::instanceCacheEnsure(instances);
+    if (rc == TRHIP_OK) rc = ctx.cl->dev->ensureAhead();
+    if (rc == TRHIP_OK && ctx.cl->dev->ahead.stream) rc = instances->cullCache.allocateAlt(ctx.cl->dev, numRecords * kInstanceCacheTransformBytesPerInstance);
+    if (rc != TRHIP_OK) return rc;
+    auto overlapped = std::make_shared<bool>(false);
+    auto fn = [=](hipStream_t s) {
         const uint64_t now = instances->version;
-        const trhip::Stamp was = instances->cullCache.built;
+        trhip::DerivedData& cc = instances->cullCache;
+        const trhip::Stamp was = cc.built;
         const bool refresh = was.other && was.version + 1 == now && !getenv("TRHIP_NO_CACHE_REFRESH");
-        const InstanceCullCache cache = refresh ? instanceCacheLayout(instances->cullCache.ptr, instances->byteSize / sizeof(BasePassInstanceConstants)) : InstanceCullCache{};
+        InstanceCullCache cache = {};
+        if (refresh && *overlapped) {
+            trhip_buffer_t::CullGenLevel& lv = instances->cullGenLevel;
+            if (!lv.level || lv.first != first || lv.count != n || lv.mapVersion != primToNode->version) {
+                TRHIP_HIP(hipMemcpyAsync(cc.spare(), cc.live(), numRecords * kInstanceCacheTransformBytesPerInstance, hipMemcpyDeviceToDevice, s));
+                lv = { true, first, n, primToNode->version };
+            }
+            cache = instanceCacheLayout(cc.ptr, numRecords, cc.spare());
+        } else if (refresh) {
+            cache = instanceCacheLayout(cc.ptr, numRecords, cc.live());
+        }
         TRHIP_LAUNCH(updateInstanceConstsKernel, dim3((n + kUpdBlock - 1) / kUpdBlock), dim3(kUpdBlock), 0, s, np, numNodes, pn, ip, first, n, refresh, cache);
-        if (refresh) instances->cullCache.markBuilt({ now, was.other, was.otherVersion });
-        return trhip::launchStatus("updateInstanceConstsKernel"); });
+        if (refresh) cc.markBuilt({ now, was.other, was.otherVersion });
+        if (refresh && *overlapped) cc.altLive = !cc.altLive;
+        return trhip::launchStatus("updateInstanceConstsKernel"); };
+    *overlapped = ctx.emitAhead("main", std::move(fn), { { instances->ptr, true }, { nodes->ptr, false }, { primToNode->ptr, false },
+                                                          { instances->cullCache.ptr, false }, { nullptr, true, &instances->cullCache } });
     return TRHIP_OK;
 }
 
diff --git a/toyrenderer_amd/csrc/trhip_core.cpp b/toyrenderer_amd/csrc/trhip_core.cpp
--- a/toyrenderer_amd/csrc/trhip_core.cpp
+++ b/toyrenderer_amd/csrc/trhip_core.cpp
@@ -104,6 +104,15 @@
     for (const Op::Access& t : touched) if (t.ptr) cl->ops.back().touched.push_back(t);
 }
 
+bool DispatchCtx::emitAhead(const char* kernelName, std::function<int(hipStream_t)> fn, std::initializer_list<Op::Access> touched) const
+{
+    emit(kernelName, std::move(fn));
+    if (cl->dev->ensureAhead() != TRHIP_OK || !cl->dev->ahead.stream) return false;
+    cl->ops.back().lane = 2;
+    for (const Op::Access& t : touched) if (t.ptr || t.gen) cl->ops.back().touched.push_back(t);
+    return true;
+}
+
 }
 
 using namespace trhip;
@@ -178,6 +187,38 @@
 {
     TRHIP_HIP(hipStreamSynchronize(stream));
     if (sideStream) TRHIP_HIP(hipStreamSynchronize(sideStream));
+    if (ahead.stream) TRHIP_HIP(hipStreamSynchronize(ahead.stream));
+    return TRHIP_OK;
+}
+
+int trhip_device_t::ensureAhead()
+{
+    std::lock_guard<std::mutex> lock(mutex);
+    if (ahead.stream || !sideStream) return TRHIP_OK;
+    TRHIP_HIP(hipSetDevice(index));
+    int lowest = 0, highest = 0;
+    TRHIP_HIP(hipDeviceGetStreamPriorityRange(&lowest, &highest));
+    for (hipEvent_t& e : ahead.runDone) TRHIP_HIP(hipEventCreateWithFlags(&e, hipEventDisableTiming));
+    TRHIP_HIP(hipStreamCreateWithPriority(&ahead.stream, hipStreamNonBlocking, lowest));
+    return TRHIP_OK;
+}
+
+int trhip_device_t::joinAhead(hipStream_t s)
+{
+    if (!ahead.stream) return TRHIP_OK;
+    if (ahead.runCounter) TRHIP_HIP(hipStreamWaitEvent(s, ahead.runDone[ahead.runCounter % kSideRuns], 0));
+    aheadNotBefore = mainSerial;
+    return TRHIP_OK;
+}
+
+int trhip::DerivedData::allocateAlt(const trhip_device_t* dev, uint64_t size)
+{
+    if (alt) return size <= altBytes ? TRHIP_OK : fail(TRHIP_ERR_STATE, "second generation of %llu bytes asked to grow to %llu", (unsigned long long)altBytes, (unsigned long long)size);
+    TRHIP_HIP(hipSetDevice(dev->index));
+    void* p = nullptr;
+    TRHIP_HIP(hipMalloc(&p, (size_t)size));
+    alt = p;
+    altBytes = size;
     return TRHIP_OK;
 }
 
@@ -195,12 +236,14 @@
 void trhip::freeDerived(trhip_device_t* dev, std::initializer_list<DerivedData*> all)
 {
     bool any = false;
-    for (const DerivedData* d : all) any |= d->ptr != nullptr;
+    for (const DerivedData* d : all) any |= d->ptr != nullptr || d->alt != nullptr;
     if (!any) return;
     (void)hipSetDevice(dev->index);
     (void)dev->syncAll();
-    for (const DerivedData* d : all)
+    for (const DerivedData* d : all) {
         if (d->ptr) (void)hipFree(d->ptr);
+        if (d->alt) (void)hipFree(d->alt);
+    }
 }
 
 void trhip_cmdlist_t::resetRecording()
@@ -313,8 +356,9 @@
         int lowest = 0, highest = 0;
         TRHIP_HIP(hipDeviceGetStreamPriorityRange(&lowest, &highest));
         TRHIP_HIP(hipStreamCreateWithPriority(&dev->sideStream, hipStreamNonBlocking, highest));
-        TRHIP_HIP(hipEventCreateWithFlags(&dev->evFork, hipEventDisableTiming));
-        for (hipEvent_t& e : dev->runDone) TRHIP_HIP(hipEventCreateWithFlags(&e, hipEventDisableTiming));
+        dev->side.stream = dev->sideStream;
+        for (hipEvent_t& e : dev->forkEv) TRHIP_HIP(hipEventCreateWithFlags(&e, hipEventDisableTiming));
+        for (hipEvent_t& e : dev->side.runDone) TRHIP_HIP(hipEventCreateWithFlags(&e, hipEventDisableTiming));
     }
     *out = dev.release();
     return TRHIP_OK;
@@ -331,8 +375,10 @@
     (void)dev->drainProfile();
     for (hipEvent_t e : dev->eventPool) (void)hipEventDestroy(e);
     if (dev->sideStream) { (void)hipStreamSynchronize(dev->sideStream); (void)hipStreamDestroy(dev->sideStream); }
-    if (dev->evFork) (void)hipEventDestroy(dev->evFork);
-    for (hipEvent_t e : dev->runDone) if (e) (void)hipEventDestroy(e);
+    if (dev->ahead.stream) (void)hipStreamDestroy(dev->ahead.stream);
+    for (hipEvent_t e : dev->forkEv) if (e) (void)hipEventDestroy(e);
+    for (hipEvent_t e : dev->side.runDone) if (e) (void)hipEventDestroy(e);
+    for (hipEvent_t e : dev->ahead.runDone) if (e) (void)hipEventDestroy(e);
     if (dev->srgbTable.ptr) (void)hipFree(dev->srgbTable.ptr);
     if (dev->ownsStream) (void)hipStreamDestroy(dev->stream);
     delete dev;
@@ -350,10 +396,13 @@
     if (!dev) return fail(TRHIP_ERR_INVALID, "device is null");
     TRHIP_HIP(hipSetDevice(dev->index));
     std::lock_guard<std::mutex> lock(dev->mutex);
-    if (dev->sideStream && dev->sideRunCounter > dev->mainWaitedUpTo) {
-        TRHIP_HIP(hipStreamWaitEvent(dev->stream, dev->runDone[dev->sideRunCounter % trhip_device_t::kSideRuns], 0));
-        dev->mainWaitedUpTo = dev->sideRunCounter;
-    }
+    for (trhip_device_t::Lane* l : { &dev->side, &dev->ahead })
+        if (l->stream && l->runCounter > l->mainWaitedUpTo) {
+            TRHIP_HIP(hipStreamWaitEvent(dev->stream, l->runDone[l->runCounter % trhip_device_t::kSideRuns], 0));
+            l->mainWaitedUpTo = l->runCounter;
+            l->mainWaitedAt = dev->mainSerial + 1;
+        }
+    dev->aheadNotBefore = dev->mainSerial + 1;
     return TRHIP_OK;
 }
 
@@ -600,6 +649,10 @@
 {
     if (!b) return fail(TRHIP_ERR_INVALID, "buffer_mark_written: null argument");
     b->version.fetch_add(1);
+    if (b->dev) {
+        std::lock_guard<std::mutex> lock(b->dev->mutex);
+        b->dev->aheadNotBefore = b->dev->mainSerial + 1;
+    }
     return TRHIP_OK;
 }
 
@@ -1124,38 +1177,44 @@
     if (!dev || (n && !lists)) return fail(TRHIP_ERR_INVALID, "queue_execute: null argument");
     TRHIP_HIP(hipSetDevice(dev->index));
     std::lock_guard<std::mutex> lock(dev->mutex);
-    bool inRun = false;
-    std::vector<Op::Access> runTouched;
-    auto endRun = [&]() -> int {
-        if (!inRun) return TRHIP_OK;
-        inRun = false;
-        const uint64_t id = ++dev->sideRunCounter;
-        const uint32_t slot = (uint32_t)(id % trhip_device_t::kSideRuns);
-        if (id > trhip_device_t::kSideRuns && id - trhip_device_t::kSideRuns > dev->mainWaitedUpTo) {
-            TRHIP_HIP(hipStreamWaitEvent(dev->stream, dev->runDone[slot], 0));
-            dev->mainWaitedUpTo = id - trhip_device_t::kSideRuns;
+    using Lane = trhip_device_t::Lane;
+    constexpr uint32_t kRuns = trhip_device_t::kSideRuns, kForks = trhip_device_t::kForks;
+    struct OpenRun { Lane* lane; bool open = false; std::vector<Op::Access> touched; };
+    OpenRun sideRun{ &dev->side }, aheadRun{ &dev->ahead };
+    auto endRun = [&](OpenRun& r) -> int {
+        if (!r.open) return TRHIP_OK;
+        r.open = false;
+        Lane& l = *r.lane;
+        const uint64_t id = ++l.runCounter;
+        const uint32_t slot = (uint32_t)(id % kRuns);
+        if (id > kRuns && id - kRuns > l.mainWaitedUpTo) {
+            TRHIP_HIP(hipStreamWaitEvent(dev->stream, l.runDone[slot], 0));
+            l.mainWaitedUpTo = id - kRuns;
+            l.mainWaitedAt = dev->mainSerial + 1;
         }
-        TRHIP_HIP(hipEventRecord(dev->runDone[slot], dev->sideStream));
-        for (const Op::Access& t : runTouched) (t.write ? dev->sideWriter : dev->sideReader)[t.ptr] = id;
-        runTouched.clear();
+        TRHIP_HIP(hipEventRecord(l.runDone[slot], l.stream));
+        for (const Op::Access& t : r.touched) (t.write ? l.writer : l.reader)[t.ptr] = id;
+        r.touched.clear();
         return TRHIP_OK;
     };
-    auto ownerOf = [&](const void* ptr, bool write) -> uint64_t {
+    auto ownerOf = [&](const Lane& l, const void* ptr, bool write) -> uint64_t {
         uint64_t need = 0;
-        auto w = dev->sideWriter.find(ptr);
-        if (w != dev->sideWriter.end()) need = w->second;
+        auto w = l.writer.find(ptr);
+        if (w != l.writer.end()) need = w->second;
         if (write) {
-            auto r = dev->sideReader.find(ptr);
-            if (r != dev->sideReader.end() && r->second > need) need = r->second;
+            auto r = l.reader.find(ptr);
+            if (r != l.reader.end() && r->second > need) need = r->second;
         }
         return need;
     };
-    auto waitForRun = [&](uint64_t need) -> int {
-        if (need <= dev->mainWaitedUpTo) return TRHIP_OK;
-        TRHIP_HIP(hipStreamWaitEvent(dev->stream, dev->runDone[need % trhip_device_t::kSideRuns], 0));
-        dev->mainWaitedUpTo = need;
+    auto waitForRun = [&](Lane& l, uint64_t need) -> int {
+        if (need <= l.mainWaitedUpTo) return TRHIP_OK;
+        TRHIP_HIP(hipStreamWaitEvent(dev->stream, l.runDone[need % kRuns], 0));
+        l.mainWaitedUpTo = need;
+        l.mainWaitedAt = dev->mainSerial;
         return TRHIP_OK;
     };
+    auto takeFork = [&](uint64_t serial) { dev->forkSerial[dev->forkCount % kForks] = serial; ++dev->forkCount; };
     auto nextIsSide = [&](uint32_t li, size_t oi) -> bool {
         if (!dev->sideStream) return false;
         for (++oi; li < n; ++li, oi = 0)
@@ -1171,28 +1230,85 @@
         for (size_t oi = 0; oi < cl->ops.size(); ++oi) {
             const Op& op = cl->ops[oi];
             const bool side = op.lane == 1 && dev->sideStream;
+            const bool ahead = op.lane == 2 && dev->ahead.stream;
             hipStream_t stream = dev->stream;
             if (side) {
-                if (!inRun) {
-                    if (!dev->forkSignalled) TRHIP_HIP(hipEventRecord(dev->evFork, dev->stream));
+                int rc = endRun(aheadRun);
+                if (rc != TRHIP_OK) return rc;
+                if (!sideRun.open) {
+                    if (!dev->forkSignalled) {
+                        TRHIP_HIP(hipEventRecord(dev->forkEv[dev->forkCount % kForks], dev->stream));
+                        takeFork(dev->mainSerial);
+                    }
                     dev->forkSignalled = false;
-                    TRHIP_HIP(hipStreamWaitEvent(dev->sideStream, dev->evFork, 0));
-                    inRun = true;
+                    TRHIP_HIP(hipStreamWaitEvent(dev->sideStream, dev->forkEv[(dev->forkCount - 1) % kForks], 0));
+                    sideRun.open = true;
                 }
-                runTouched.insert(runTouched.end(), op.touched.begin(), op.touched.end());
+                for (const Op::Access& t : op.touched) {
+                    const uint64_t need = ownerOf(dev->ahead, t.ptr, t.write);
+                    if (need > dev->ahead.mainWaitedUpTo) TRHIP_HIP(hipStreamWaitEvent(dev->sideStream, dev->ahead.runDone[need % kRuns], 0));
+                }
+                sideRun.touched.insert(sideRun.touched.end(), op.touched.begin(), op.touched.end());
                 stream = dev->sideStream;
                 for (; mark < cl->useMarks.size() && cl->useMarks[mark].op <= oi; ++mark)
                     if (cl->useMarks[mark].write && cl->useMarks[mark].version) cl->useMarks[mark].version->fetch_add(1);
+            } else if (ahead) {
+                int rc = endRun(sideRun);
+                if (rc != TRHIP_OK) return rc;
+                uint64_t required = dev->aheadNotBefore;
+                for (Op::Access t : op.touched) {
+                    if (t.gen) t.ptr = t.gen->spare();
+                    if (!t.ptr) continue;
+                    auto seen = dev->mainTouch.find(t.ptr);
+                    if (seen == dev->mainTouch.end())
+                        seen = dev->mainTouch.emplace(t.ptr, trhip_device_t::Touch{ dev->mainSerial, dev->mainSerial }).first;
+                    required = std::max(required, seen->second.write);
+                    if (t.write) required = std::max(required, seen->second.read);
+                    const uint64_t need = ownerOf(dev->side, t.ptr, t.write);
+                    if (need > dev->side.mainWaitedUpTo) TRHIP_HIP(hipStreamWaitEvent(dev->ahead.stream, dev->side.runDone[need % kRuns], 0));
+                    else if (need) required = std::max(required, dev->side.mainWaitedAt);
+                    aheadRun.touched.push_back(t);
+                }
+                if (required > dev->aheadForkedAt) {
+                    const uint64_t have = std::min<uint64_t>(dev->forkCount, kForks);
+                    uint64_t best = UINT64_MAX, bestSlot = 0;
+                    for (uint64_t k = 0; k < have; ++k) {
+                        const uint64_t slot = (dev->forkCount - 1 - k) % kForks;
+                        if (dev->forkSerial[slot] >= required && dev->forkSerial[slot] < best) { best = dev->forkSerial[slot]; bestSlot = slot; }
+                    }
+                    if (best == UINT64_MAX) {
+                        bestSlot = dev->forkCount % kForks;
+                        TRHIP_HIP(hipEventRecord(dev->forkEv[bestSlot], dev->stream));
+                        takeFork(dev->mainSerial);
+                        dev->forkSignalled = false;
+                        best = dev->mainSerial + 1;
+                    }
+                    TRHIP_HIP(hipStreamWaitEvent(dev->ahead.stream, dev->forkEv[bestSlot], 0));
+                    dev->aheadForkedAt = best;
+                }
+                aheadRun.open = true;
+                stream = dev->ahead.stream;
+                for (; mark < cl->useMarks.size() && cl->useMarks[mark].op <= oi; ++mark)
+                    if (cl->useMarks[mark].write && cl->useMarks[mark].version) cl->useMarks[mark].version->fetch_add(1);
             } else {
-                int rc = endRun();
+                int rc = endRun(sideRun);
+                if (rc == TRHIP_OK) rc = endRun(aheadRun);
                 if (rc != TRHIP_OK) return rc;
-                uint64_t need = 0;
+                const uint64_t serial = ++dev->mainSerial;
+                uint64_t need = 0, needAhead = 0;
                 for (; mark < cl->useMarks.size() && cl->useMarks[mark].op <= oi; ++mark) {
                     const trhip_cmdlist_t::UseMark& m = cl->useMarks[mark];
-                    need = std::max(need, ownerOf(m.ptr, m.write));
+                    const void* ptr = m.gen ? m.gen->live() : m.ptr;
+                    need = std::max(need, ownerOf(dev->side, ptr, m.write));
+                    if (dev->ahead.stream) {
+                        needAhead = std::max(needAhead, ownerOf(dev->ahead, ptr, m.write));
+                        auto seen = dev->mainTouch.find(ptr);
+                        if (seen != dev->mainTouch.end()) (m.write ? seen->second.write : seen->second.read) = serial;
+                    }
                     if (m.write && m.version) m.version->fetch_add(1);
                 }
-                rc = waitForRun(need);
+                rc = waitForRun(dev->side, need);
+                if (rc == TRHIP_OK) rc = waitForRun(dev->ahead, needAhead);
                 if (rc != TRHIP_OK) return rc;
             }
             const bool prof = dev->profiling && !op.name.empty() && (dev->profileFilter.empty() || dev->profileFilter == op.name);
@@ -1200,18 +1316,19 @@
             if (prof) { e0 = dev->acquireEvent(); e1 = dev->acquireEvent(); TRHIP_HIP(hipEventRecord(e0, stream)); }
             const auto h0 = g_hostProfile.on ? std::chrono::steady_clock::now() : std::chrono::steady_clock::time_point{};
             trhip::LaunchTap tap;
-            dev->forkSignalled = false;
-            const bool tapped = !side && !prof && strcmp(op.kind, "host_callback") != 0 && nextIsSide(i, oi);
-            if (tapped) { tap.onStream = stream; tap.stopEvent = dev->evFork; trhip::g_launchTap = &tap; }
+            if (!side && !ahead) dev->forkSignalled = false;
+            const bool tapped = !side && !ahead && !prof && strcmp(op.kind, "host_callback") != 0 && nextIsSide(i, oi);
+            if (tapped) { tap.onStream = stream; tap.stopEvent = dev->forkEv[dev->forkCount % kForks]; trhip::g_launchTap = &tap; }
             int rc = op.fn(stream);
             trhip::g_launchTap = nullptr;
-            if (tapped && tap.launches >= 1 && rc == TRHIP_OK) dev->forkSignalled = true;
+            if (tapped && tap.launches >= 1 && rc == TRHIP_OK) { takeFork(dev->mainSerial); dev->forkSignalled = true; }
             if (g_hostProfile.on) g_hostProfile.add(op.kind, std::chrono::duration<double, std::micro>(std::chrono::steady_clock::now() - h0).count());
             if (rc != TRHIP_OK) return rc;
             if (prof) { TRHIP_HIP(hipEventRecord(e1, stream)); dev->pending.push_back({ op.name, e0, e1 }); }
         }
     }
-    return endRun();
+    int rc = endRun(sideRun);
+    return rc == TRHIP_OK ? endRun(aheadRun) : rc;
 }
 
 int trhip_stream_create_priority(int device_index, int priority_class, void** out)
diff --git a/toyrenderer_amd/csrc/trhip_internal.h b/toyrenderer_amd/csrc/trhip_internal.h
--- a/toyrenderer_amd/csrc/trhip_internal.h
+++ b/toyrenderer_amd/csrc/trhip_internal.h
@@ -65,6 +65,13 @@
     int allocate(const trhip_device_t* dev, uint64_t size);
     bool current(const Stamp& s) const { return built == s; }
     void markBuilt(const Stamp& s) { built = s; }
+
+    void* alt = nullptr;
+    uint64_t altBytes = 0;
+    bool altLive = false;
+    int allocateAlt(const trhip_device_t* dev, uint64_t size);
+    void* live() const { return altLive ? alt : ptr; }
+    void* spare() const { return altLive ? ptr : alt; }
 };
 
 }
@@ -80,13 +87,30 @@
 
     static constexpr uint32_t kSideRuns = 16;
     hipStream_t sideStream = nullptr;
-    hipEvent_t evFork = nullptr;
     bool forkSignalled = false;
-    hipEvent_t runDone[kSideRuns] = {};
-    uint64_t sideRunCounter = 0;
-    uint64_t mainWaitedUpTo = 0;
-    std::unordered_map<const void*, uint64_t> sideWriter;
-    std::unordered_map<const void*, uint64_t> sideReader;
+    struct Lane
+    {
+        hipStream_t stream = nullptr;
+        hipEvent_t runDone[kSideRuns] = {};
+        uint64_t runCounter = 0;
+        uint64_t mainWaitedUpTo = 0;
+        uint64_t mainWaitedAt = 0;
+        std::unordered_map<const void*, uint64_t> writer;
+        std::unordered_map<const void*, uint64_t> reader;
+    };
+    Lane side;
+    static constexpr uint32_t kForks = 16;
+    Lane ahead;
+    hipEvent_t forkEv[kForks] = {};
+    uint64_t forkSerial[kForks] = {};
+    uint64_t forkCount = 0;
+    uint64_t mainSerial = 0;
+    uint64_t aheadForkedAt = 0;
+    uint64_t aheadNotBefore = 0;
+    struct Touch { uint64_t read = 0, write = 0; };
+    std::unordered_map<const void*, Touch> mainTouch;
+    int ensureAhead();
+    int joinAhead(hipStream_t s);
     int syncAll();
 
     std::mutex mutex;
@@ -131,6 +155,7 @@
     std::vector<uint8_t> shadow;
     std::atomic<uint64_t> version{1};
     trhip::DerivedData cullCache;
+    struct CullGenLevel { bool level = false; uint32_t first = 0, count = 0; uint64_t mapVersion = 0; } cullGenLevel;
     trhip::DerivedData cullStream;
     trhip::DerivedData triCounts;
     trhip::DerivedData order;
@@ -199,7 +224,7 @@
     std::function<int(hipStream_t)> fn;
     const char* kind = "dispatch";
     uint8_t lane = 0;
-    struct Access { const void* ptr; bool write; };
+    struct Access { const void* ptr; bool write; const DerivedData* gen = nullptr; };
     std::vector<Access> touched;
 };
 
@@ -238,12 +263,12 @@
     int recordClearWords(void* ptr, uint64_t words, uint32_t value, bool fresh = false);
     bool usedSoFar(const void* ptr) const { for (const UseMark& m : useMarks) if (m.ptr == ptr) return true; return false; }
 
-    struct UseMark { size_t op; const void* ptr; bool write; std::atomic<uint64_t>* version; };
+    struct UseMark { size_t op; const void* ptr; bool write; std::atomic<uint64_t>* version; const trhip::DerivedData* gen; };
     std::vector<UseMark> useMarks;
-    void use(const void* ptr, size_t op, bool write, std::atomic<uint64_t>* version = nullptr)
+    void use(const void* ptr, size_t op, bool write, std::atomic<uint64_t>* version = nullptr, const trhip::DerivedData* gen = nullptr)
     {
         if (!ptr) return;
-        useMarks.push_back({ op, ptr, write, version });
+        useMarks.push_back({ op, ptr, write, version, gen });
     }
     void forgetUse(const void* ptr, size_t op)
     {
@@ -283,12 +308,14 @@
     void* scratchSide(size_t bytes) const { return cl->dev->sideStream ? cl->scratchAllocSide(bytes) : cl->scratchAlloc(bytes); }
     void emit(const char* kernelName, std::function<int(hipStream_t)> fn) const;
     void emitSide(const char* kernelName, std::function<int(hipStream_t)> fn, std::initializer_list<Op::Access> touched) const;
+    bool emitAhead(const char* kernelName, std::function<int(hipStream_t)> fn, std::initializer_list<Op::Access> touched) const;
 };
 
 int hzbQuadEnsure(trhip_texture_t* tex);
 int hzbQuadLaunchBuild(trhip_texture_t* tex, hipStream_t s);
 
 int instanceCacheEnsure(trhip_buffer_t* instances);
+void instanceCacheUse(trhip_cmdlist_t* cl, trhip_buffer_t* instances);
 int instanceCacheLaunchBuild(trhip_buffer_t* instances, trhip_buffer_t* meshData, hipStream_t s);
 
 inline uint32_t tableMinGroups()
```

After: 119.9. About the same (-0.1%).
